# PROBIC/mSWEEP

Hardware: AMD Instinct MI355X
Metric: EM iters/sec + reads×groups cells/sec, 10M reads × 5k groups (higher is better)
Workload: dtype f64

## Files before the change

### msweep_amd/csrc/common.hpp

```cpp
#pragma once
#include <hip/hip_runtime.h>

#include <cstdint>
#include <cstdio>
#include <stdexcept>
#include <string>
#include <vector>

namespace msw {

constexpr int kWave = 64;
#ifndef MSW_PASS_THREADS_A
#define MSW_PASS_THREADS_A 1024
#endif
#ifndef MSW_PASS_THREADS_B
#define MSW_PASS_THREADS_B 768
#endif
#ifndef MSW_PASS_THREADS_B8
#define MSW_PASS_THREADS_B8 1024
#endif
constexpr int kPassThreads = MSW_PASS_THREADS_A;
constexpr int kPassThreadsB = MSW_PASS_THREADS_B;
constexpr int kPassThreadsB8 = MSW_PASS_THREADS_B8;
constexpr int kMaxTrace = 4096;
constexpr int kRedfinParts = 5;
constexpr int kRedfinGroups = 16;
#ifndef MSW_REDFIN_THREADS
#define MSW_REDFIN_THREADS 512
#endif
constexpr int kRedfinThreads = MSW_REDFIN_THREADS;
constexpr int kRedfinSlots = kRedfinThreads / kRedfinGroups;
#ifndef MSW_FX
#define MSW_FX 1
#endif
constexpr bool kFx = MSW_FX != 0;

struct HipError : std::runtime_error {
  using std::runtime_error::runtime_error;
};

#define MSW_HIP(expr)                                                                      \
  do {                                                                                     \
    hipError_t _e = (expr);                                                                \
    if (_e != hipSuccess) {                                                                \
      char _b[512];                                                                        \
      snprintf(_b, sizeof _b, "%s failed: %s (%s:%d)", #expr, hipGetErrorString(_e),       \
               __FILE__, __LINE__);                                                        \
      throw ::msw::HipError(_b);                                                           \
    }                                                                                      \
  } while (0)

template <class T>
struct DevBuf {
  T *p = nullptr;
  size_t n = 0;
  DevBuf() = default;
  DevBuf(const DevBuf &) = delete;
  DevBuf &operator=(const DevBuf &) = delete;
  ~DevBuf() { release(); }
  void release() {
    if (p) (void)hipFree(p);
    p = nullptr;
    n = 0;
  }
  void alloc(size_t count) {
    if (count <= n && p) return;
    release();
    if (count == 0) count = 1;
    MSW_HIP(hipMalloc((void **)&p, count * sizeof(T)));
    n = count;
  }
  void upload(const T *src, size_t count, hipStream_t s) {
    alloc(count);
    if (count) MSW_HIP(hipMemcpyAsync(p, src, count * sizeof(T), hipMemcpyHostToDevice, s));
  }
  void zero(hipStream_t s) {
    if (p) MSW_HIP(hipMemsetAsync(p, 0, n * sizeof(T), s));
  }
};

struct SolveOpts {
  int32_t check_every = 1;
  double init_bound = -100000.0;
  int32_t em_prior = 0;
  int32_t em_stop = 0;
};

#ifdef MSW_STAMPS
__device__ unsigned long long g_stamps[64 * 40];
#define MSW_STAMP(it, K, p) (g_stamps[((it) & 63) * 40 + (K) * 8 + (p)] = __builtin_amdgcn_s_memrealtime())
#define MSW_STAMP_MAX(it, K, p) atomicMax(&g_stamps[((it) & 63) * 40 + (K) * 8 + (p)], (unsigned long long)__builtin_amdgcn_s_memrealtime())
#else
#define MSW_STAMP(it, K, p) ((void)0)
#define MSW_STAMP_MAX(it, K, p) ((void)0)
#endif

struct TabDev {
  double2 *A, *B;
};

struct Scalars {
  double a, os_a, step_a;
  double oldnorm, newnorm, beta;
  double bound, oldbound, bound_const;
  double tol, csum;
  double M, U, p0, kappa;
  double logzi;
  double fx_scale, fx_inv, fx_tscale, fx_tinv, xb, tmax, tmin;
  double tref;
  int32_t didreset, reset_pending, done, iter;
  int32_t have_eval, eval_pad;
  int32_t max_iters, fixed_iters, trace_theta, flavor;
  int32_t check_every, em_prior, em_stop, opt_pad;
  int32_t tab_ver, fx_shift;
};

}
```

### msweep_amd/csrc/msweep_core.hip

```cpp
#include "../../include/msweep_core.h"

#include <algorithm>
#include <array>
#include <cmath>
#include <chrono>
#include <cstring>
#include <limits>
#include <memory>
#include <string>
#include <thread>
#include <unordered_map>
#include <vector>

#include <rocprim/device/device_radix_sort.hpp>
#include <rocprim/device/device_scan.hpp>
#include <rocprim/iterator/counting_iterator.hpp>
#include <rocprim/iterator/transform_iterator.hpp>

#include "kernels.hpp"
#include "pack_kernels.hpp"
#include "compress_kernels.hpp"
#include "comm.hpp"
#include "shm_comm.hpp"
#include "peer_comm.hpp"
#include "likelihood_kernels.hpp"
#include "bootstrap_kernels.hpp"
#include "em_kernels.hpp"
#include "em_f32_kernels.hpp"
#include "stream_kernels.hpp"
#include "reader_kernels.hpp"
#include "bin_kernels.hpp"

using namespace msw;

namespace {
thread_local std::string g_create_error;
constexpr size_t kLdsMax = 160 * 1024;
constexpr int kIterBatch = 16;
}


struct LikShape {
  int flavor = -1;
  uint32_t G = 0, E = 0, n_lut = 0, nslices = 0, n_long = 0;
  uint64_t nnz = 0, nslots = 0;
  int enc = kEncNarrow;
  bool glds = true, tlds = true;
  int gmodeB = 1;
  RecDec dec = {};
  uint32_t n_area = 0;
  uint32_t n_tab_lds = 0;
  SliceClasses cls = {};
  bool packed_scheduled = false;
  uint32_t long_row = kLongRow;
  uint64_t rows_over8 = 0;
  bool passB_rc8 = false;
  double logzi = 0.0;
  int nblk = 0;
  int nblk_dense = 0;
  int nreg = 0;
  bool have_logc_res = false;
};

struct Resident : LikShape {
  DevBuf<uint32_t> rec, slice_off, long_ptr, rec_long, perm;
  DevBuf<uint8_t> slice_hot;
  DevBuf<uint32_t> area_slot;
  DevBuf<double> lut_area;
  DevBuf<double> lut, Lt;
  DevBuf<double> trange;
  DevBuf<double> logc_res;
  bool wide() const { return enc == kEncWide; }
  bool hybrid() const { return enc == kEncIndex; }
  int n_tab_inline() const { return flavor == 0 && n_area <= (uint32_t)kTabInline ? (int)n_area : 0; }
  int npart_rows() const { return flavor == 0 ? nblk : (nreg >= 32 ? 4 * nblk_dense : nblk_dense); }
  uint32_t guard_cap() const {
    static_assert(kPassThreads / 64 <= 16 && kPassThreadsB / 64 <= 16, "guard_cap / guard_bits assume <= 16 wavefronts per workgroup");
    const uint32_t nb0 = (uint32_t)std::max(nblk, 1);
    return 64u * ((nslices + nb0 - 1) / nb0 + 16u) + (n_long + nb0 - 1) / nb0 + 16u;
  }
  uint32_t guard_words() const { return (G + 31u) / 32u; }
};

struct Solver {
  hipStream_t stream = nullptr;
  int n_cu = 256;
  msw_comm *const *commp;
  bool *collective;
  explicit Solver(msw_comm *const *c = nullptr, bool *coll = nullptr) : commp(c), collective(coll) {}
  msw_comm *comm() const { return commp ? *commp : nullptr; }
  SolveOpts opts;
  bool profiling = false, fixed_iters = false;
  size_t trace_theta = 0;

  DevBuf<double> cvec, logc_d, alpha0, u, os_u, step_u, w, e, N, Nc, Acc;
  DevBuf<uint8_t> c8, c8s;
  DevBuf<double2> ew, tabA, tabB;
  TabDev tabs() const { return TabDev{tabA.p, tabB.p}; }
  DevBuf<int> tab_built;
  DevBuf<double> partA, partS, partAcc, partC, partR, totS;
  size_t lds_attr[3][80] = {};
  DevBuf<double> commA, commB;
  DevBuf<uint32_t> guard_list, guard_bits;
  DevBuf<unsigned long long> guard_tail;
  DevBuf<int> guard_err;
  DevBuf<unsigned long long> guard_visits;
  DevBuf<Scalars> sc;
  Scalars *sc_host = nullptr;
  DevBuf<double> tr_bound, tr_newnorm, tr_beta, tr_theta;
  DevBuf<int32_t> tr_reset;
  bool have_solution = false;
  bool prepared = false;
  int last_algo = MSW_ALGO_RCG;
  DevBuf<double> logth;
  DevBuf<float> e32, tab32;
  bool em_f32 = false;

  msw_timing timing = {};
  hipEvent_t ev0 = nullptr, ev1 = nullptr;
  std::vector<std::pair<hipEvent_t, hipEvent_t>> evA, evB, evC;
  size_t evA_used = 0, evB_used = 0, evC_used = 0;

  ~Solver() {
    if (sc_host) (void)hipHostFree(sc_host);
    if (ev0) (void)hipEventDestroy(ev0);
    if (ev1) (void)hipEventDestroy(ev1);
    for (auto &p : evA) { (void)hipEventDestroy(p.first); (void)hipEventDestroy(p.second); }
    for (auto &p : evB) { (void)hipEventDestroy(p.first); (void)hipEventDestroy(p.second); }
    for (auto &p : evC) { (void)hipEventDestroy(p.first); (void)hipEventDestroy(p.second); }
  }
};

struct Resampler {
  DevBuf<uint64_t> mtwords;
  DevBuf<uint32_t> bcounts, bcounts2;
  DevBuf<MtState> mt;
  hipStream_t stream2 = nullptr;
  hipEvent_t ev_counts[2] = {nullptr, nullptr};
  uint32_t one_count = 0;
  bool mt_valid = false;
  int32_t mt_seed = 0;
  uint64_t mt_pos = 0;
  ~Resampler() {
    for (auto &e : ev_counts)
      if (e) (void)hipEventDestroy(e);
    if (stream2) (void)hipStreamDestroy(stream2);
  }
};

struct Worker {
  Solver s;
  Resampler r;
  explicit Worker(int n_cu) { MSW_HIP(hipStreamCreateWithFlags(&s.stream, hipStreamNonBlocking)); s.n_cu = n_cu; }
  ~Worker() { (void)hipStreamDestroy(s.stream); }
};

struct msw_core {
  int device = 0;
  int n_cu = 256;
  hipStream_t stream = nullptr;
  std::string err;
  TextStager text_stage;
  ReaderPool reader_pool;
  msw_comm *comm = nullptr;
  bool in_collective = false;
  bool pack_schedule = true;
  bool no_hybrid = false;

  Resident lik;
  DevBuf<uint32_t> iperm;
  Solver solver{&comm, &in_collective};

  DevBuf<double> cp;
  std::vector<uint32_t> cp_counts;
  bool cp_hit = false;
  Resampler resampler;
  std::vector<std::unique_ptr<Worker>> workers;
  msw_bootstrap_timing btiming = {};

  ~msw_core() { if (stream) (void)hipStreamDestroy(stream); }
};

namespace {

struct Fail : std::runtime_error {
  using std::runtime_error::runtime_error;
};
struct NumericFail : Fail {
  using Fail::Fail;
};

struct CollectiveScope {
  bool *flag;
  explicit CollectiveScope(bool *f) : flag(f) { if (flag) *flag = true; }
  void leave() { if (flag) *flag = false; }
};

template <class F>
int guarded(msw_handle h, F &&f) {
  if (!h) return 1;
  try {
    MSW_HIP(hipSetDevice(h->device));
    f();
    return 0;
  } catch (const std::exception &ex) {
    h->err = ex.what();
    (void)hipGetLastError();
    if (h->comm && h->in_collective) h->comm->abort();
    h->in_collective = false;
    return 1;
  }
}

std::pair<hipEvent_t, hipEvent_t> &next_pair(std::vector<std::pair<hipEvent_t, hipEvent_t>> &v,
                                             size_t &used) {
  if (used == v.size()) {
    hipEvent_t a, b;
    MSW_HIP(hipEventCreate(&a));
    MSW_HIP(hipEventCreate(&b));
    v.emplace_back(a, b);
  }
  return v[used++];
}

SellDev sell_view(const Resident &L, const Solver &s) {
  SellDev S;
  S.rec = L.rec.p;
  S.slice_off = L.slice_off.p;
  S.long_ptr = L.long_ptr.p;
  S.rec_long = L.rec_long.p;
  S.perm = L.perm.p;
  S.cvec = s.cvec.p;
  S.c8 = s.c8.p;
  S.c8s = s.c8s.p;
  S.nslices = L.nslices;
  S.n_long = L.n_long;
  S.n_ecs = L.E;
  S.n_groups = L.G;
  S.n_lut = L.n_lut;
  S.n_area = L.n_area;
  S.area_slot = L.area_slot.p;
  S.shift = L.dec.shift;
  S.mask = L.dec.mask;
  S.bhi = L.dec.bhi;
  S.bhiA = L.dec.bhiA;
  S.shiftH = L.dec.shiftH;
  S.maskH = L.dec.maskH;
  S.n_tab_lds = L.n_tab_lds;
  S.slice_hot = L.slice_hot.p;
  S.lut_area = L.lut_area.p;
  S.cls = L.cls;
  return S;
}
GuardDev guard_view(const Resident &L, const Solver &s) {
  return GuardDev{s.guard_list.p, s.guard_bits.p, s.guard_tail.p, L.lut_area.p, s.guard_err.p, s.guard_visits.p, L.guard_cap(),
                  L.guard_words()};
}

int passB_mode(const Resident &L, bool glds, uint32_t n_tab, bool index) {
  const uint32_t G = L.G;
  if (glds) {
    if (pass_lds_bytes(1, n_tab, G, false, index) > kLdsMax) return -1;
    if (8ull * (G + kSentinels) <= kAccFixed && pass_lds_bytes(2, n_tab, G, false, index) <= kLdsMax) return 2;
    return 1;
  }
  if (pass_lds_bytes(0, n_tab, G, false, index) > kLdsMax) return -1;
  if (getenv("MSWEEP_GLOBAL_ATOMICS")) return 0;
  if (pass_lds_bytes(3, n_tab, G, false, index) <= kLdsMax) return 3;
  if (pass_lds_bytes(4, n_tab, G, false, index) <= kLdsMax) return 4;
  return 0;
}

bool multilane() {
  const char *e = getenv("MSWEEP_MULTILANE");
  return !(e && atoi(e) == 0);
}
SliceClasses make_slice_classes(const uint32_t *n) {
  SliceClasses C = {};
  for (int c = 0; c < kSliceClasses; ++c) {
    const uint32_t per = 64u >> (kMaxLgm - c);
    C.p0[c + 1] = C.p0[c] + n[c];
    C.s0[c + 1] = C.s0[c] + (n[c] + per - 1) / per;
  }
  return C;
}

void choose_lds_mode(Resident &L) {
  const bool opts[4][2] = {{true, true}, {true, false}, {false, true}, {false, false}};
  const char *force = getenv("MSWEEP_FORCE_LDS");
  for (auto &o : opts) {
    if (force && strlen(force) == 2 && (o[0] != (force[0] == '1') || o[1] != (force[1] == '1'))) continue;
    const uint32_t n_tab = o[1] ? L.n_area : 0u;
    const int gmB = passB_mode(L, o[0], n_tab, false);
    if (!force && !o[0] && o[1] && gmB == 0 && !getenv("MSWEEP_GLOBAL_ATOMICS")) continue;
    if (gmB >= 0 && pass_lds_bytes(o[0] ? 1 : 0, n_tab, L.G, true, false) <= kLdsMax) {
      L.glds = o[0];
      L.tlds = o[1];
      L.gmodeB = gmB;
      L.n_tab_lds = n_tab;
      return;
    }
  }
  throw Fail("internal: no LDS configuration fits");
}

void choose_layout(Resident &L) {
  choose_lds_mode(L);
  L.dec.bhi = sell_bhi(L.n_tab_lds);
  L.dec.bhiA = 2 * L.dec.bhi;
  const uint64_t lo_end = 16ull * std::max<uint32_t>(L.n_area, 1);
  const uint64_t hi_end = (uint64_t)L.dec.bhi + 8ull * ((uint64_t)L.G + kSentinels);
  L.enc = kEncWide;
  L.dec.shift = 0;
  L.dec.mask = 0xffffffffu;
  const char *force = getenv("MSWEEP_RECORD_BYTES");
  for (uint32_t s = 5; s <= 31 && !(force && atoi(force) == 8); ++s) {
    if (lo_end <= (1ull << (s - 1)) && hi_end <= (1ull << (32 - s))) {
      L.enc = kEncNarrow;
      L.dec.shift = s;
      L.dec.mask = (1u << (s - 1)) - 1u;
      break;
    }
  }
  if (L.wide() && (hi_end > (1ull << 31) || lo_end > (1ull << 32)))
    throw Fail("likelihood too large: group / lookup-table offsets exceed the 8-byte record fields");
}

bool choose_hybrid_layout(Resident &L, bool no_hybrid) {
  if (L.tlds || no_hybrid) return false;
  if (const char *e = getenv("MSWEEP_HYBRID"))
    if (atoi(e) == 0) return false;
  const char *force = getenv("MSWEEP_RECORD_BYTES");
  if (force && atoi(force) == 8) return false;
  uint32_t eb = 1, gb = 1;
  while ((1ull << eb) < std::max<uint32_t>(L.n_area, 2)) ++eb;
  while ((1ull << gb) < (uint64_t)L.G + kSentinels) ++gb;
  if (eb + gb > 32) return false;
  uint32_t n_hot = 0;
  {
    const int gmA = L.glds ? 1 : 0;
    uint32_t lo = 0, hi = std::min<uint32_t>(L.n_area, (uint32_t)(kLdsMax / 16)) / 16;
    while (lo < hi) {
      const uint32_t mid = (lo + hi + 1) / 2, n = mid * 16;
      const bool ok = pass_lds_bytes(gmA, n, L.G, true, true) <= kLdsMax && passB_mode(L, L.glds, n, true) >= 0 &&
                      (L.glds || passB_mode(L, false, n, true) == passB_mode(L, false, 0, true));
      if (ok) lo = mid;
      else hi = mid - 1;
    }
    n_hot = lo * 16;
  }
  if (const char *e = getenv("MSWEEP_HYBRID_HOT")) n_hot = std::min<uint32_t>(n_hot, (uint32_t)atoi(e) & ~15u);
  L.enc = kEncIndex;
  L.dec.shift = eb;
  L.dec.mask = (1u << eb) - 1u;
  L.n_tab_lds = std::min(n_hot, L.n_area);
  uint32_t hb = 4;
  while ((1ull << hb) < 16ull * std::max<uint32_t>(L.n_tab_lds, 1)) ++hb;
  if (hb + gb > 32) return false;
  L.dec.shiftH = hb;
  L.dec.maskH = (1u << hb) - 1u;
  L.dec.bhi = L.dec.bhiA = sell_bhi(L.n_tab_lds);
  L.gmodeB = passB_mode(L, L.glds, L.n_tab_lds, true);
  return true;
}

void alloc_solve_state(const Resident &L, Solver &s) {
  const uint32_t G = L.G, E = L.E;
  for (DevBuf<double> *b : {&s.alpha0, &s.u, &s.os_u, &s.step_u, &s.w, &s.e, &s.N, &s.Nc,
                            &s.Acc, &s.logth})
    b->alloc((size_t)G + kSentinels);
  s.ew.alloc((size_t)G + kSentinels);
  s.e.zero(s.stream);
  s.ew.zero(s.stream);
  s.cvec.alloc(E);
  s.c8.alloc((size_t)E + 64);
  s.c8s.alloc((size_t)L.nslices * 64 + 64);
  s.c8s.zero(s.stream);
  s.logc_d.alloc(E);
  s.tabA.alloc((size_t)std::max<uint32_t>(L.n_area, 1));
  s.tabB.alloc((size_t)std::max<uint32_t>(L.n_area, 1));
  s.tab_built.alloc(2);
  const int nb = std::max(L.nblk, std::max(L.nblk_dense, L.npart_rows()));
  s.partA.alloc(std::max(nb, 1024));
  s.partS.alloc(4 * (size_t)std::max(nb, 1024));
  s.partR.alloc(kRedfinParts * ((size_t)G / kRedfinGroups + 2));
  s.totS.alloc(4);
  s.commA.alloc(1);
  s.commB.alloc(3 * (size_t)G + 4);
  s.partAcc.alloc((size_t)std::max(nb, 1) * G);
  s.partC.alloc(1024);
  if (L.flavor == 0) {
    const uint32_t nb0 = (uint32_t)std::max(L.nblk, 1);
    s.guard_list.alloc((size_t)nb0 * L.guard_cap());
    s.guard_bits.alloc((size_t)nb0 * 16 * L.guard_words());
    s.guard_bits.zero(s.stream);
    s.guard_tail.alloc(2 * (size_t)G);
    s.guard_tail.zero(s.stream);
  }
  s.guard_err.alloc(1);
  s.guard_err.zero(s.stream);
  s.guard_visits.alloc(1);
  s.guard_visits.zero(s.stream);
  s.sc.alloc(1);
  s.tr_bound.alloc(kMaxTrace);
  s.tr_newnorm.alloc(kMaxTrace);
  s.tr_beta.alloc(kMaxTrace);
  s.tr_reset.alloc(kMaxTrace);
  if (!s.sc_host) MSW_HIP(hipHostMalloc((void **)&s.sc_host, sizeof(Scalars)));
  if (!s.ev0) {
    MSW_HIP(hipEventCreate(&s.ev0));
    MSW_HIP(hipEventCreate(&s.ev1));
  }
}

template <class K>
void prepare_sweep(K k, size_t lds, size_t &lds_set) {
  if (lds > lds_set) {
    hipFuncAttributes fa;
    MSW_HIP(hipFuncGetAttributes(&fa, (const void *)k));
    if (fa.sharedSizeBytes != 0) throw Fail("internal: sweep kernel owns static LDS");
    MSW_HIP(hipFuncSetAttribute((const void *)k, hipFuncAttributeMaxDynamicSharedMemorySize, (int)lds));
    lds_set = lds;
  }
}
template <int ENC, bool GL, bool TL>
void launch_passA_t(const Resident &L, Solver &s) {
  const size_t lds = pass_lds_bytes(GL ? 1 : 0, L.n_tab_lds, L.G, true, ENC == kEncIndex);
  const bool ml = L.cls.s0[kSliceClasses - 1] > 0;
  auto k = ml ? k_passA<ENC, GL, TL, true> : k_passA<ENC, GL, TL, false>;
  prepare_sweep(k, lds, s.lds_attr[0][(ml ? 40 : 0) + ENC * 4 + (GL ? 2 : 0) + (TL ? 1 : 0)]);
  hipLaunchKernelGGL(k, dim3(L.nblk), dim3(pass_threads_A<ENC>()), lds, s.stream, s.sc.p, sell_view(L, s),
                     s.ew.p, s.tabA.p, s.partA.p, s.partR.p, (int)((L.G + kRedfinGroups - 1) / kRedfinGroups),
                     guard_view(L, s));
}
template <int ENC, int GM, bool TL>
void launch_passB_t(const Resident &L, Solver &s) {
  const size_t lds = pass_lds_bytes(GM, L.n_tab_lds, L.G, false, ENC == kEncIndex);
  const bool ml = L.cls.s0[kSliceClasses - 1] > 0;
  if constexpr (ENC == kEncNarrow) {
    if (L.passB_rc8 && !ml) {
      auto k8 = k_passB<ENC, GM, TL, false, 8>;
      prepare_sweep(k8, lds, s.lds_attr[2][2 * GM + (TL ? 1 : 0)]);
      const auto rg_of = [&](uint32_t g0) {
        return GM == 4 ? RangeB{g0, std::min<uint32_t>(kRangeGroups, L.G - g0), g0 == 0 ? 1 : 0} : RangeB{0, 0, 1};
      };
      for (uint32_t g0 = 0; g0 < (GM == 4 ? L.G : 1u); g0 += kRangeGroups)
        hipLaunchKernelGGL(k8, dim3(L.nblk), dim3(pass_threads_B<ENC, 8>()), lds, s.stream, s.sc.p, sell_view(L, s), s.e.p,
                           s.tabB.p, s.partAcc.p, s.partS.p, s.Acc.p, rg_of(g0), guard_view(L, s));
      return;
    }
  }
  auto k = ml ? k_passB<ENC, GM, TL, true> : k_passB<ENC, GM, TL, false>;
  prepare_sweep(k, lds, s.lds_attr[1][(ml ? 40 : 0) + ENC * 10 + 2 * GM + (TL ? 1 : 0)]);
  if (GM == 4) {
    for (uint32_t g0 = 0; g0 < L.G; g0 += kRangeGroups)
      hipLaunchKernelGGL(k, dim3(L.nblk), dim3(pass_threads_B<ENC>()), lds, s.stream, s.sc.p, sell_view(L, s), s.e.p,
                         s.tabB.p, s.partAcc.p, s.partS.p, s.Acc.p,
                         RangeB{g0, std::min<uint32_t>(kRangeGroups, L.G - g0), g0 == 0 ? 1 : 0}, guard_view(L, s));
    return;
  }
  hipLaunchKernelGGL(k, dim3(L.nblk), dim3(pass_threads_B<ENC>()), lds, s.stream, s.sc.p, sell_view(L, s), s.e.p,
                     s.tabB.p, s.partAcc.p, s.partS.p, s.Acc.p, RangeB{0, 0, 1}, guard_view(L, s));
}

#define MSW_DISPATCH3(fn, ...)                                                       \
  do {                                                                               \
    const int key = L.enc * 4 + (L.glds ? 2 : 0) + (L.tlds ? 1 : 0);              \
    switch (key) {                                                                   \
      case 0: fn<kEncNarrow, false, false>(__VA_ARGS__); break;                      \
      case 1: fn<kEncNarrow, false, true>(__VA_ARGS__); break;                       \
      case 2: fn<kEncNarrow, true, false>(__VA_ARGS__); break;                       \
      case 3: fn<kEncNarrow, true, true>(__VA_ARGS__); break;                        \
      case 4: fn<kEncWide, false, false>(__VA_ARGS__); break;                        \
      case 5: fn<kEncWide, false, true>(__VA_ARGS__); break;                         \
      case 6: fn<kEncWide, true, false>(__VA_ARGS__); break;                         \
      case 7: fn<kEncWide, true, true>(__VA_ARGS__); break;                          \
      case 8: fn<kEncIndex, false, false>(__VA_ARGS__); break;                       \
      case 10: fn<kEncIndex, true, false>(__VA_ARGS__); break;                       \
      case 12: fn<kEncValue, false, false>(__VA_ARGS__); break;                      \
      case 14: fn<kEncValue, true, false>(__VA_ARGS__); break;                       \
      default: throw Fail("internal: no sweep for this layout");                     \
    }                                                                                \
  } while (0)
#define MSW_DISPATCH_B(fn, ...)                                                      \
  do {                                                                               \
    const int key = L.enc * 10 + 2 * L.gmodeB + (L.tlds ? 1 : 0);                 \
    switch (key) {                                                                   \
      case 0: fn<kEncNarrow, 0, false>(__VA_ARGS__); break;                          \
      case 1: fn<kEncNarrow, 0, true>(__VA_ARGS__); break;                           \
      case 2: fn<kEncNarrow, 1, false>(__VA_ARGS__); break;                          \
      case 3: fn<kEncNarrow, 1, true>(__VA_ARGS__); break;                           \
      case 4: fn<kEncNarrow, 2, false>(__VA_ARGS__); break;                          \
      case 5: fn<kEncNarrow, 2, true>(__VA_ARGS__); break;                           \
      case 6: fn<kEncNarrow, 3, false>(__VA_ARGS__); break;                          \
      case 7: fn<kEncNarrow, 3, true>(__VA_ARGS__); break;                           \
      case 8: fn<kEncNarrow, 4, false>(__VA_ARGS__); break;                          \
      case 9: fn<kEncNarrow, 4, true>(__VA_ARGS__); break;                           \
      case 10: fn<kEncWide, 0, false>(__VA_ARGS__); break;                           \
      case 11: fn<kEncWide, 0, true>(__VA_ARGS__); break;                            \
      case 12: fn<kEncWide, 1, false>(__VA_ARGS__); break;                           \
      case 13: fn<kEncWide, 1, true>(__VA_ARGS__); break;                            \
      case 14: fn<kEncWide, 2, false>(__VA_ARGS__); break;                           \
      case 15: fn<kEncWide, 2, true>(__VA_ARGS__); break;                            \
      case 16: fn<kEncWide, 3, false>(__VA_ARGS__); break;                           \
      case 17: fn<kEncWide, 3, true>(__VA_ARGS__); break;                            \
      case 18: fn<kEncWide, 4, false>(__VA_ARGS__); break;                           \
      case 19: fn<kEncWide, 4, true>(__VA_ARGS__); break;                            \
      case 20: fn<kEncIndex, 0, false>(__VA_ARGS__); break;                          \
      case 22: fn<kEncIndex, 1, false>(__VA_ARGS__); break;                          \
      case 24: fn<kEncIndex, 2, false>(__VA_ARGS__); break;                          \
      case 26: fn<kEncIndex, 3, false>(__VA_ARGS__); break;                          \
      case 28: fn<kEncIndex, 4, false>(__VA_ARGS__); break;                          \
      case 30: fn<kEncValue, 0, false>(__VA_ARGS__); break;                          \
      case 32: fn<kEncValue, 1, false>(__VA_ARGS__); break;                          \
      case 34: fn<kEncValue, 2, false>(__VA_ARGS__); break;                          \
      case 36: fn<kEncValue, 3, false>(__VA_ARGS__); break;                          \
      case 38: fn<kEncValue, 4, false>(__VA_ARGS__); break;                          \
      default: throw Fail("internal: no sweep for this layout");                     \
    }                                                                                \
  } while (0)

template <int NREG>
void launch_dense_A(const Resident &L, Solver &s) {
  hipLaunchKernelGGL(k_dense_passA<NREG>, dim3(L.nblk_dense), dim3(256), 0, s.stream, s.sc.p,
                     L.Lt.p, (int)L.G, L.E, s.u.p, s.w.p, s.partA.p);
}
template <int NREG>
void launch_dense_B(const Resident &L, Solver &s) {
  const size_t lds = (32 + 4 * (size_t)L.G) * sizeof(double);
  hipLaunchKernelGGL(k_dense_passB<NREG>, dim3(L.nblk_dense), dim3(256), lds, s.stream, s.sc.p,
                     L.Lt.p, (int)L.G, L.E, s.cvec.p, s.u.p, s.partAcc.p, s.partS.p);
}
template <int NREG>
void launch_dense_big_A(const Resident &L, Solver &s) {
  hipLaunchKernelGGL(k_dense_big_passA<NREG>, dim3(L.nblk_dense), dim3(256), 0, s.stream, s.sc.p,
                     L.Lt.p, (int)L.G, L.E, s.u.p, s.w.p, s.partA.p);
}
template <int NREG>
void launch_dense_big_B(const Resident &L, Solver &s) {
  hipLaunchKernelGGL(k_dense_big_passB<NREG>, dim3(L.nblk_dense), dim3(256), 0, s.stream, s.sc.p,
                     L.Lt.p, (int)L.G, L.E, s.cvec.p, s.u.p, s.partAcc.p, s.partS.p);
}
#define MSW_DISPATCH_NREG(fn, fnbig, ...)                \
  do {                                                   \
    switch (L.nreg) {                                   \
      case 1: fn<1>(__VA_ARGS__); break;                 \
      case 2: fn<2>(__VA_ARGS__); break;                 \
      case 4: fn<4>(__VA_ARGS__); break;                 \
      case 8: fn<8>(__VA_ARGS__); break;                 \
      case 16: fn<16>(__VA_ARGS__); break;               \
      case 32: fnbig<32>(__VA_ARGS__); break;            \
      case 64: fnbig<64>(__VA_ARGS__); break;            \
      default: fnbig<128>(__VA_ARGS__); break;           \
    }                                                    \
  } while (0)

void launch_passA(const Resident &L, Solver &s) {
  std::pair<hipEvent_t, hipEvent_t> *ev = nullptr;
  if (s.profiling) {
    ev = &next_pair(s.evA, s.evA_used);
    MSW_HIP(hipEventRecord(ev->first, s.stream));
  }
  if (L.flavor == 0) MSW_DISPATCH3(launch_passA_t, L, s);
  else MSW_DISPATCH_NREG(launch_dense_A, launch_dense_big_A, L, s);
  MSW_HIP(hipGetLastError());
  if (ev) MSW_HIP(hipEventRecord(ev->second, s.stream));
  s.timing.passA_launches++;
}

bool em_f32_layout_ok(const Resident &L, const Solver &s) {
  if (!kFx || L.flavor != 0 || !L.glds || s.comm() || L.G > (uint32_t)(kStepRegs * 1024)) return false;
  if (getenv("MSWEEP_EM_FLOAT_AS_DOUBLE")) return false;
  if (L.enc == kEncNarrow)
    return L.tlds && L.n_tab_lds == L.n_area && em_f32_lds_bytes(L.n_tab_lds, L.G) <= kLdsMax;
  if (L.hybrid()) return L.dec.shift <= 30 && em_f32_idx_lds_bytes(L.n_area, L.G) <= kLdsMax;
  return false;
}
void launch_em_passB_f32(const Resident &L, Solver &s) {
  const bool idx = L.hybrid();
  const size_t lds = idx ? em_f32_idx_lds_bytes(L.n_area, L.G) : em_f32_lds_bytes(L.n_tab_lds, L.G);
  const bool ml = L.cls.s0[kSliceClasses - 1] > 0;
  auto k = idx ? (ml ? k_em_passB_f32_idx<true> : k_em_passB_f32_idx<false>)
               : (ml ? k_em_passB_f32<true> : k_em_passB_f32<false>);
  prepare_sweep(k, lds, s.lds_attr[2][30 + (idx ? 2 : 0) + (ml ? 1 : 0)]);
  hipLaunchKernelGGL(k, dim3(L.nblk), dim3(1024), lds, s.stream, s.sc.p, sell_view(L, s), s.e.p, s.e32.p, s.tab32.p,
                     s.partAcc.p, s.partS.p, guard_view(L, s));
}

void launch_passB(const Resident &L, Solver &s) {
  std::pair<hipEvent_t, hipEvent_t> *ev = nullptr;
  if (s.profiling) {
    ev = &next_pair(s.evB, s.evB_used);
    MSW_HIP(hipEventRecord(ev->first, s.stream));
  }
  if (L.flavor == 0 && s.em_f32) {
    launch_em_passB_f32(L, s);
  } else if (L.flavor == 0) {
    if (L.gmodeB == 0) MSW_HIP(hipMemsetAsync(s.Acc.p, 0, ((size_t)L.G + kSentinels) * sizeof(double), s.stream));
    MSW_DISPATCH_B(launch_passB_t, L, s);
  } else {
    MSW_DISPATCH_NREG(launch_dense_B, launch_dense_big_B, L, s);
  }
  MSW_HIP(hipGetLastError());
  if (ev) MSW_HIP(hipEventRecord(ev->second, s.stream));
  s.timing.passB_launches++;
  const bool partials = (L.flavor == 1) || L.gmodeB > 0 || s.em_f32;
  const int nb = L.npart_rows();
  const int fxrows = L.flavor == 0 ? (s.em_f32 ? 2 : 1) : 0;
  if (s.comm()) {
    const size_t G3 = 3 * (size_t)L.G;
    std::pair<hipEvent_t, hipEvent_t> *evc = nullptr;
    if (s.profiling) {
      evc = &next_pair(s.evC, s.evC_used);
      MSW_HIP(hipEventRecord(evc->first, s.stream));
    }
    hipLaunchKernelGGL(k_colsum, dim3((L.G + 63) / 64), dim3(1024), 0, s.stream, s.sc.p, (int)L.G,
                       partials ? nb : 0, fxrows, nb, s.partAcc.p, s.Acc.p, s.partS.p,
                       fxrows ? s.guard_tail.p : nullptr, s.commB.p);
    if (kFx && fxrows) {
      s.comm()->allreduce_mixed(reinterpret_cast<uint64_t *>(s.commB.p), G3, s.commB.p + G3, 4, s.stream);
    } else {
      s.comm()->allreduce(s.commB.p, (size_t)L.G, s.stream);
      s.comm()->allreduce_mixed(reinterpret_cast<uint64_t *>(s.commB.p) + L.G, 2 * (size_t)L.G, s.commB.p + G3, 4,
                               s.stream);
    }
    if (evc) MSW_HIP(hipEventRecord(evc->second, s.stream));
    hipLaunchKernelGGL(k_redfin, dim3((L.G + kRedfinGroups - 1) / kRedfinGroups), dim3(kRedfinThreads), 0, s.stream,
                       s.sc.p, (int)L.G, 0, fxrows, reinterpret_cast<unsigned long long *>(s.commB.p) + L.G, 0, 1,
                       s.partAcc.p, s.commB.p, s.commB.p + G3, s.e.p, s.u.p,
                       s.alpha0.p, s.Nc.p, s.N.p, s.w.p, s.ew.p, s.partR.p, s.totS.p);
    return;
  }
  hipLaunchKernelGGL(k_redfin, dim3((L.G + kRedfinGroups - 1) / kRedfinGroups), dim3(kRedfinThreads), 0, s.stream,
                     s.sc.p, (int)L.G, partials ? nb : 0, fxrows, fxrows ? s.guard_tail.p : nullptr, 1, nb,
                     s.partAcc.p, s.Acc.p, s.partS.p, s.e.p,
                     s.u.p, s.alpha0.p, s.Nc.p, s.N.p, s.w.p, s.ew.p, s.partR.p, s.totS.p);
}

const double *fin_partS(const Resident &L, Solver &s) { return s.comm() ? s.commB.p + 3 * (size_t)L.G : s.partS.p; }
int fin_npartS(const Resident &L, Solver &s) { return s.comm() ? 1 : L.npart_rows(); }

void launch_tables(const Resident &L, Solver &s) {
  if (L.flavor != 0 || L.n_area <= (uint32_t)kTabInline) return;
  const unsigned nb = std::min<unsigned>((L.n_area + 255) / 256, (unsigned)s.n_cu * 8);
  hipLaunchKernelGGL(k_tables, dim3(nb), dim3(256), 0, s.stream, s.sc.p, (int)L.n_area, L.lut_area.p, s.tabs(),
                     s.tab_built.p);
}

void launch_finstep(const Resident &L, Solver &s, int mode) {
  TraceDev tr{s.tr_bound.p, s.tr_newnorm.p, s.tr_beta.p, s.tr_theta.p, s.tr_reset.p};
  const double *pA = s.partA.p;
  int npA = L.flavor == 0 ? L.nblk : L.nblk_dense;
  if (s.comm()) {
    pA = s.commA.p;
    npA = 1;
  }
  hipLaunchKernelGGL(k_finstep, dim3(1), dim3(1024), 0, s.stream, s.sc.p, mode, (int)L.G, L.n_tab_inline(), npA, pA,
                     (int)((L.G + kRedfinGroups - 1) / kRedfinGroups), s.totS.p, s.partR.p, s.Nc.p, s.w.p, s.u.p,
                     s.os_u.p, s.step_u.p, L.lut_area.p, s.e.p, s.tabs(), tr);
  launch_tables(L, s);
}

void poll(Solver &s) {
  MSW_HIP(hipMemcpyAsync(s.sc_host, s.sc.p, sizeof(Scalars), hipMemcpyDeviceToHost, s.stream));
  MSW_HIP(hipStreamSynchronize(s.stream));
  if (s.comm()) s.comm()->check();
}

constexpr int kCvecBlocks = 512;
void prepare_inputs(const Resident &L, Solver &s, const double *logc_host, const uint32_t *counts_dev,
                    const double *alpha0_host) {
  if (L.flavor < 0) throw Fail("no likelihood resident: call msw_core_set_csr / set_dense_logl first");
  const uint32_t E = L.E, G = L.G;
  if (counts_dev) {
    hipLaunchKernelGGL(k_cvec_from_counts, dim3(kCvecBlocks), dim3(256), 0, s.stream, counts_dev,
                       L.flavor == 0 ? L.perm.p : nullptr, E, s.cvec.p, s.c8.p, s.partC.p, L.cls, L.n_long,
                       L.flavor == 0 ? s.c8s.p : nullptr);
  } else {
    const double *src = s.logc_d.p;
    if (logc_host) {
      MSW_HIP(hipMemcpyAsync(s.logc_d.p, logc_host, E * sizeof(double), hipMemcpyHostToDevice, s.stream));
    } else {
      if (!L.have_logc_res) throw Fail("null logc: only a likelihood built by msw_core_build_likelihood keeps its log counts");
      src = L.logc_res.p;
    }
    hipLaunchKernelGGL(k_cvec_from_logc, dim3(kCvecBlocks), dim3(256), 0, s.stream, src,
                       L.flavor == 0 ? L.perm.p : nullptr, E, s.cvec.p, s.c8.p, s.partC.p, L.cls, L.n_long,
                       L.flavor == 0 ? s.c8s.p : nullptr);
  }
  if (alpha0_host)
    MSW_HIP(hipMemcpyAsync(s.alpha0.p, alpha0_host, G * sizeof(double), hipMemcpyHostToDevice, s.stream));
  MSW_HIP(hipGetLastError());
  MSW_HIP(hipStreamSynchronize(s.stream));
  s.prepared = true;
}

void validate_solve(size_t max_iters, int algo, int prec) {
  if (algo != MSW_ALGO_RCG && algo != MSW_ALGO_EM) throw Fail("unknown algorithm id");
  if (prec != MSW_PREC_DOUBLE && prec != MSW_PREC_FLOAT) throw Fail("unknown precision id");
  if (max_iters == 0 || max_iters > (size_t)std::numeric_limits<int32_t>::max())
    throw Fail("max_iters out of range");
}

void begin_solve(const Resident &L, Solver &s, double tol, size_t max_iters) {
  const uint32_t G = L.G;
  if (s.trace_theta) s.tr_theta.alloc(s.trace_theta * G);
  const double *cpart = s.partC.p;
  int ncpart = kCvecBlocks;
  if (s.comm()) {
    s.comm()->rendezvous();
    hipLaunchKernelGGL(k_sum_scalar, dim3(1), dim3(1024), 0, s.stream, s.sc.p, 0, kCvecBlocks, s.partC.p,
                       s.commA.p);
    s.comm()->allreduce(s.commA.p, 1, s.stream);
    cpart = s.commA.p;
    ncpart = 1;
  }
  hipLaunchKernelGGL(k_init_state, dim3(1), dim3(1024), 0, s.stream, s.sc.p, (int)G, ncpart,
                     cpart, s.alpha0.p, s.u.p, s.os_u.p, s.step_u.p, tol, (int)max_iters,
                     s.fixed_iters ? 1 : 0, (int)s.trace_theta, L.flavor, L.logzi, s.opts, s.tab_built.p,
                     L.trange.p);
  MSW_HIP(hipGetLastError());
}

void run_rcg(const Resident &L, Solver &s, size_t max_iters, size_t iters_start = 0) {
  const int G = (int)L.G, n_lut = L.n_tab_inline();
  if (iters_start > 0 && s.comm()) s.comm()->rendezvous();
  if (iters_start == 0) {
    hipLaunchKernelGGL(k_prepB, dim3(1), dim3(1024), 0, s.stream, s.sc.p, G, n_lut, s.u.p, L.lut_area.p,
                       s.e.p, s.tabs());
    launch_tables(L, s);
    launch_passB(L, s);
    s.timing.passB_launches--;
    if (s.profiling && s.evB_used) s.evB_used--;
  }
  const int nbA = L.flavor == 0 ? L.nblk : L.nblk_dense;
  size_t iters_done = iters_start;
  for (;;) {
    const size_t missing = std::max<size_t>(1, max_iters - std::min(max_iters, iters_done));
    const size_t batch = s.fixed_iters ? std::min<size_t>(256, missing) : std::min<size_t>(kIterBatch, missing);
    for (size_t b = 0; b < batch; ++b) {
      launch_passA(L, s);
      if (s.comm()) {
        std::pair<hipEvent_t, hipEvent_t> *evc = nullptr;
        if (s.profiling) {
          evc = &next_pair(s.evC, s.evC_used);
          MSW_HIP(hipEventRecord(evc->first, s.stream));
        }
        hipLaunchKernelGGL(k_sum_scalar, dim3(1), dim3(1024), 0, s.stream, s.sc.p, 1, nbA, s.partA.p,
                           s.commA.p);
        s.comm()->allreduce(s.commA.p, 1, s.stream);
        if (evc) MSW_HIP(hipEventRecord(evc->second, s.stream));
      }
      launch_finstep(L, s, 0);
      launch_passB(L, s);
    }
    MSW_HIP(hipGetLastError());
    poll(s);
    if (s.sc_host->done) break;
    if (s.sc_host->have_eval && (size_t)s.sc_host->iter + 1 >= max_iters) {
      launch_finstep(L, s, 1);
      MSW_HIP(hipGetLastError());
      poll(s);
      if (s.sc_host->done) break;
    }
    iters_done = (size_t)s.sc_host->iter;
  }
}

void finish_solve(const Resident &L, Solver &s, double *theta_out, size_t *iters_out, double *bound_out) {
  poll(s);
  const uint32_t G = L.G;
  int gerr = 0;
  MSW_HIP(hipMemcpy(&gerr, s.guard_err.p, sizeof gerr, hipMemcpyDeviceToHost));
  if (gerr) {
    MSW_HIP(hipMemset(s.guard_err.p, 0, sizeof gerr));
    if (gerr == 2) throw Fail("internal: a workgroup's list of guarded equivalence classes overflowed");
    throw NumericFail("likelihood underflow: an equivalence class has zero probability under every group "
                      "(exp(a * log-likelihood) and the group weights underflow fp64 together)");
  }
  if (s.sc_host->iter > 0 && !std::isfinite(s.sc_host->bound))
    throw NumericFail("the evidence lower bound is not finite: the likelihood or the prior counts are out of range");
  if (theta_out) {
    if (s.last_algo == MSW_ALGO_EM) {
      MSW_HIP(hipMemcpy(theta_out, s.logth.p, G * sizeof(double), hipMemcpyDeviceToHost));
    } else {
      std::vector<double> nc(G);
      MSW_HIP(hipMemcpy(nc.data(), s.Nc.p, G * sizeof(double), hipMemcpyDeviceToHost));
      const double csum = s.sc_host->csum;
      for (uint32_t g = 0; g < G; ++g) theta_out[g] = nc[g] / csum;
    }
  }
  if (iters_out) *iters_out = (size_t)s.sc_host->iter;
  if (bound_out) *bound_out = s.sc_host->bound;
  s.have_solution = true;
}

void collect_timing(const Resident &L, Solver &s) {
  float ms = 0.f;
  MSW_HIP(hipEventElapsedTime(&ms, s.ev0, s.ev1));
  s.timing.solve_ms = ms;
  s.timing.passA_ms = s.timing.passB_ms = 0.0;
  if (s.profiling) {
    for (size_t i = 0; i < s.evA_used; ++i) {
      MSW_HIP(hipEventElapsedTime(&ms, s.evA[i].first, s.evA[i].second));
      s.timing.passA_ms += ms;
    }
    for (size_t i = 0; i < s.evB_used; ++i) {
      MSW_HIP(hipEventElapsedTime(&ms, s.evB[i].first, s.evB[i].second));
      s.timing.passB_ms += ms;
    }
    s.timing.collective_ms = 0.0;
    for (size_t i = 0; i < s.evC_used; ++i) {
      MSW_HIP(hipEventElapsedTime(&ms, s.evC[i].first, s.evC[i].second));
      s.timing.collective_ms += ms;
    }
    s.timing.collectives = s.evC_used;
  }
  s.timing.iters = (uint64_t)s.sc_host->iter;
  const uint64_t recsz = L.enc == kEncValue ? 12 : (L.wide() ? 8 : 4);
  if (L.flavor == 0) {
    const uint64_t tab = L.tlds ? 0ull : 16ull * (L.n_area - L.n_tab_lds);
    s.timing.bytes_passA = L.nnz * recsz + tab;
    s.timing.bytes_passB = L.nnz * recsz + 1ull * L.E + tab;
  } else {
    s.timing.bytes_passA = 8ull * L.E * L.G;
    s.timing.bytes_passB = 8ull * L.E * L.G + 8ull * L.E;
  }
}

void run_em(const Resident &L, Solver &s, size_t max_iters, int prec);

void continue_impl(const Resident &L, Solver &s, size_t n_iters, double *theta_out, size_t *iters_out, double *bound_out) {
  if (!s.have_solution || !s.fixed_iters || s.last_algo != MSW_ALGO_RCG)
    throw Fail("msw_core_continue: needs a fixed-iteration RCG solve on the handle (msw_core_set_fixed_iters, msw_core_run)");
  const size_t start = (size_t)s.sc_host->iter;
  if (n_iters == 0 || start + n_iters > (size_t)std::numeric_limits<int32_t>::max()) throw Fail("msw_core_continue: iteration count out of range");
  s.timing = {};
  s.evA_used = s.evB_used = s.evC_used = 0;
  CollectiveScope cs(s.collective);
  hipLaunchKernelGGL(k_extend, dim3(1), dim3(1), 0, s.stream, s.sc.p, (int)n_iters);
  MSW_HIP(hipEventRecord(s.ev0, s.stream));
  run_rcg(L, s, start + n_iters, start);
  MSW_HIP(hipEventRecord(s.ev1, s.stream));
  finish_solve(L, s, theta_out, iters_out, bound_out);
  collect_timing(L, s);
  s.timing.iters = (uint64_t)s.sc_host->iter - start;
  cs.leave();
}

void run_impl(const Resident &L, Solver &s, double tol, size_t max_iters, int algo, int prec, double *theta_out,
              size_t *iters_out, double *bound_out) {
  validate_solve(max_iters, algo, prec);
  if (!s.prepared) throw Fail("msw_core_run: inputs not prepared (call msw_core_prepare)");
  s.timing = {};
  s.evA_used = s.evB_used = s.evC_used = 0;
  CollectiveScope cs(s.collective);
  begin_solve(L, s, tol, max_iters);
  MSW_HIP(hipEventRecord(s.ev0, s.stream));
  if (algo == MSW_ALGO_RCG) run_rcg(L, s, max_iters);
  else run_em(L, s, max_iters, prec);
  MSW_HIP(hipEventRecord(s.ev1, s.stream));
  s.last_algo = algo;
  finish_solve(L, s, theta_out, iters_out, bound_out);
  collect_timing(L, s);
  cs.leave();
}

}

namespace {
struct StageTimer {
  hipStream_t st;
  bool on;
  std::chrono::steady_clock::time_point t0;
  explicit StageTimer(hipStream_t s) : st(s), on(getenv("MSWEEP_BUILD_TIMING") != nullptr), t0(std::chrono::steady_clock::now()) {}
  void mark(const char *what) {
    if (!on) return;
    (void)hipStreamSynchronize(st);
    const auto t1 = std::chrono::steady_clock::now();
    fprintf(stderr, "[msweep build] %-28s %8.2f ms\n", what, std::chrono::duration<double, std::milli>(t1 - t0).count());
    t0 = t1;
  }
};
}

#include "host_likelihood.inc"
#include "host_pack.inc"
#include "host_em.inc"
#include "host_mtjump.inc"
#include "host_bootstrap.inc"
#include "host_build.inc"
#include "host_compress.inc"
#include "host_alignment.inc"
#include "host_reader.inc"
#include "host_bin.inc"

extern "C" {

#ifndef MSW_SRC_HASH
#define MSW_SRC_HASH "unhashed"
#endif
const char *msw_core_version(void) { return "msweep_core 0.2 gfx950 (HIP, wave64) src " MSW_SRC_HASH; }

const char *msw_last_error(msw_handle h) { return h ? h->err.c_str() : g_create_error.c_str(); }

int msw_core_create(int device, msw_handle *out) {
  if (!out) return 1;
  *out = nullptr;
  try {
    int n = 0;
    MSW_HIP(hipGetDeviceCount(&n));
    if (n <= 0) throw Fail("no HIP device visible: libmsweep_core has no CPU fallback");
    if (device < 0 || device >= n) throw Fail("device index out of range");
    MSW_HIP(hipSetDevice(device));
    hipDeviceProp_t prop;
    MSW_HIP(hipGetDeviceProperties(&prop, device));
    std::unique_ptr<msw_core> h(new msw_core);
    h->device = device;
    h->n_cu = prop.multiProcessorCount > 0 ? prop.multiProcessorCount : 256;
    MSW_HIP(hipStreamCreateWithFlags(&h->stream, hipStreamNonBlocking));
    h->solver.stream = h->stream;
    h->solver.n_cu = h->n_cu;
    hipLaunchKernelGGL(k_warm, dim3(1), dim3(1), 0, h->stream, (int *)nullptr);
    MSW_HIP(hipGetLastError());
    MSW_HIP(hipStreamSynchronize(h->stream));
    *out = h.release();
    return 0;
  } catch (const std::exception &ex) {
    g_create_error = ex.what();
    (void)hipGetLastError();
    return 1;
  }
}

void msw_core_destroy(msw_handle h) {
  if (!h) return;
  (void)hipSetDevice(h->device);
  if (h->stream) (void)hipStreamSynchronize(h->stream);
  delete h;
}

int msw_core_shape(msw_handle h, size_t *n_groups, size_t *n_ecs, size_t *nnz) {
  return guarded(h, [&] {
    if (h->lik.flavor < 0) throw Fail("no likelihood resident");
    if (n_groups) *n_groups = h->lik.G;
    if (n_ecs) *n_ecs = h->lik.E;
    if (nnz) *nnz = h->lik.flavor == 0 ? h->lik.nnz : (size_t)h->lik.G * h->lik.E;
  });
}

int msw_core_set_dense_logl(msw_handle h, const double *L, size_t n_groups, size_t n_ecs, size_t ld) {
  return guarded(h, [&] { set_dense_impl(h, L, n_groups, n_ecs, ld); });
}

int msw_core_set_csr(msw_handle h, const uint64_t *rowptr, const uint32_t *grp, const uint32_t *cnt,
                     const double *lut, size_t lut_ld, double logzi, size_t n_groups, size_t n_ecs) {
  return guarded(h, [&] { set_csr_impl(h, rowptr, grp, cnt, lut, lut_ld, logzi, n_groups, n_ecs); });
}

int msw_core_build_likelihood(msw_handle h, const uint64_t *ec_tptr, const uint32_t *ec_targets,
                              size_t n_ecs, const uint32_t *target_group, size_t n_targets,
                              const uint64_t *group_sizes, size_t n_groups, const uint64_t *ec_counts,
                              double q, double e, double zero_inflation, size_t min_hits,
                              size_t *n_groups_out, uint8_t *mask_out, double *logc_out) {
  return guarded(h, [&] {
    build_likelihood_impl(h, ec_tptr, ec_targets, n_ecs, target_group, n_targets, group_sizes,
                          n_groups, ec_counts, q, e, zero_inflation, min_hits, n_groups_out, mask_out,
                          logc_out, false, 0);
  });
}

int msw_core_build_likelihood_aln(msw_handle h, msw_alignment_t a, const uint32_t *target_group, size_t n_targets,
                                  const uint64_t *group_sizes, size_t n_groups, double q, double e,
                                  double zero_inflation, size_t min_hits, size_t *n_groups_out, uint8_t *mask_out,
                                  double *logc_out) {
  return guarded(h, [&] {
    if (!a) throw Fail("msw_core_build_likelihood_aln: null alignment");
    if (a->on_device && a->device == h->device) {
      build_likelihood_impl(h, a->d_tptr.p, a->d_targets.p, a->E, target_group, n_targets, group_sizes, n_groups,
                            a->d_counts.p, q, e, zero_inflation, min_hits, n_groups_out, mask_out, logc_out, true, a->H);
    } else {
      a->to_host(msw_alignment::kAlnTptr | msw_alignment::kAlnTargets | msw_alignment::kAlnCounts);
      build_likelihood_impl(h, a->ec_tptr.data(), a->ec_targets.data(), a->ec_counts.size(), target_group, n_targets,
                            group_sizes, n_groups, a->ec_counts.data(), q, e, zero_inflation, min_hits, n_groups_out,
                            mask_out, logc_out, false, 0);
    }
  });
}

int msw_core_trim(msw_handle h) {
  return guarded(h, [&] {
    MSW_HIP(hipStreamSynchronize(h->stream));
    h->reader_pool.trim();
  });
}

int msw_alignment_read_device(msw_handle h, const char *const *paths, size_t n_paths, size_t n_targets, int merge_mode,
                              msw_alignment_t *out) {
  if (out) *out = nullptr;
  const int rc = guarded(h, [&] {
    check_reader_args(paths, out, n_paths, n_targets, merge_mode);
    std::unique_ptr<msw_alignment> a(new msw_alignment);
    a->device = h->device;
    MSW_HIP(hipStreamSynchronize(h->stream));
    h->reader_pool.recycle();
    ReaderCtx cx(h->stream, h->n_cu, &h->text_stage, &h->reader_pool, h->device);
    bool fits = true;
    {
      uint64_t text = 0;
      for (size_t i = 0; i < n_paths; ++i) {
        struct stat sb;
        if (paths[i] && stat(paths[i], &sb) == 0) text += (uint64_t)sb.st_size * (path_is_gzip(paths[i]) ? 8u : 1u);
      }
      size_t free_b = 0, total_b = 0;
      MSW_HIP(hipMemGetInfo(&free_b, &total_b));
      const uint64_t need = 6 * text + (1ull << 30);
      if (need > (uint64_t)free_b && h->reader_pool.idle_bytes()) {
        h->reader_pool.trim();
        MSW_HIP(hipMemGetInfo(&free_b, &total_b));
      }
      fits = need <= (uint64_t)free_b + h->reader_pool.idle_bytes();
      if (getenv("MSWEEP_READER_FORCE_HOST")) fits = false;
    }
    try {
      if (!fits) throw ReaderFallback{};
      try {
        read_alignment_device(paths, n_paths, n_targets, merge_mode, cx, *a);
      } catch (const HipError &ex) {
        if (!strstr(ex.what(), "out of memory")) throw;
        (void)hipGetLastError();
        throw ReaderFallback{};
      }
    } catch (const ReaderFallback &) {
      msw_alignment_t host = nullptr;
      if (msw_alignment_read(paths, n_paths, n_targets, merge_mode, &host) != 0) throw Fail(msw_alignment_last_error());
      *out = host;
      return;
    }
    *out = a.release();
  });
  if (rc != 0 && h) g_aln_error = msw_last_error(h);
  return rc;
}

int msw_core_layout_info(msw_handle h, msw_layout_info *out) {
  return guarded(h, [&] {
    if (!out) throw Fail("null out");
    const Resident &L = h->lik;
    if (L.flavor != 0) throw Fail("msw_core_layout_info: no CSR-of-ECs likelihood resident");
    msw_layout_info li = {};
    li.record_bytes = L.enc == kEncValue ? 12 : (L.wide() ? 8 : 4);
    li.index_records = L.hybrid() ? 1 : 0;
    li.groups_in_lds = L.glds ? 1 : 0;
    li.table_in_lds = L.tlds ? 1 : 0;
    li.passB_mode = L.gmodeB;
    li.slot_entries = L.n_area;
    li.slot_entries_in_lds = L.n_tab_lds;
    li.n_slices = L.nslices;
    li.n_long_ecs = L.n_long;
    li.bank_scheduled = L.packed_scheduled ? 1 : 0;
    li.passB_reg_cells = L.passB_rc8 ? 8 : kRegCells;
    li.rows_over_8 = L.rows_over8;
    std::vector<uint32_t> off((size_t)L.nslices + 1);
    MSW_HIP(hipMemcpy(off.data(), L.slice_off.p, off.size() * sizeof(uint32_t), hipMemcpyDeviceToHost));
    li.rows = off[L.nslices];
    for (int c = 0; c < kSliceClasses; ++c) li.slices_by_lanes[c] = L.cls.s0[c + 1] - L.cls.s0[c];
    for (uint32_t s2 = 0; s2 < L.nslices; ++s2) li.max_rows = std::max(li.max_rows, off[s2 + 1] - off[s2]);
    if (L.hybrid()) {
      std::vector<uint8_t> hot(std::max<uint32_t>(L.nslices, 1));
      MSW_HIP(hipMemcpy(hot.data(), L.slice_hot.p, hot.size(), hipMemcpyDeviceToHost));
      for (uint32_t s2 = 0; s2 < L.nslices; ++s2) li.rows_from_memory += (off[s2 + 1] - off[s2]) - hot[s2];
    } else if (!L.tlds && L.enc != kEncValue) {
      li.rows_from_memory = li.rows;
    }
    *out = li;
  });
}

int msw_core_layout_hash(msw_handle h, uint64_t *hash_out) {
  return guarded(h, [&] {
    if (!hash_out) throw Fail("null out");
    *hash_out = layout_hash(h->lik);
  });
}

int msw_core_get_dense_logl(msw_handle h, double *L_out, size_t ld) {
  return guarded(h, [&] { materialise_impl(h, L_out, ld, false, 0, h->lik.E); });
}

int msw_core_gamma(msw_handle h, double *gamma_out, size_t ld) {
  return guarded(h, [&] {
    if (!h->solver.have_solution) throw Fail("msw_core_gamma: no solve has run on this handle");
    materialise_impl(h, gamma_out, ld, true, 0, h->lik.E);
  });
}

int msw_core_gamma_block(msw_handle h, size_t ec_begin, size_t ec_end, double *gamma_out, size_t ld) {
  return guarded(h, [&] {
    if (!h->solver.have_solution) throw Fail("msw_core_gamma_block: no solve has run on this handle");
    materialise_impl(h, gamma_out, ld, true, ec_begin, ec_end);
  });
}

int msw_core_bin_reads(msw_handle h, const uint64_t *ec_rptr, const uint32_t *ec_reads, size_t n_ecs,
                       const uint32_t *targets, const double *thresholds, size_t n_targets, uint64_t *bin_ptr,
                       uint32_t *reads_out, double *log_thr_out) {
  return guarded(h, [&] {
    bin_reads_impl(h, ec_rptr, ec_reads, n_ecs, false, targets, thresholds, n_targets, bin_ptr, reads_out, log_thr_out);
  });
}

int msw_core_bin_reads_aln(msw_handle h, msw_alignment_t a, const uint32_t *targets, const double *thresholds,
                           size_t n_targets, uint64_t *bin_ptr, uint32_t *reads_out, double *log_thr_out) {
  return guarded(h, [&] {
    if (!a) throw Fail("msw_core_bin_reads_aln: null alignment");
    if (a->on_device && a->device == h->device) {
      bin_reads_impl(h, a->d_rptr.p, a->d_reads.p, a->E, true, targets, thresholds, n_targets, bin_ptr, reads_out,
                     log_thr_out);
    } else {
      a->to_host(msw_alignment::kAlnRptr | msw_alignment::kAlnReads);
      bin_reads_impl(h, a->ec_rptr.data(), a->ec_reads.data(), a->ec_rptr.empty() ? 0 : a->ec_rptr.size() - 1, false,
                     targets, thresholds, n_targets, bin_ptr, reads_out, log_thr_out);
    }
  });
}

int msw_core_solve(msw_handle h, const double *logc, const double *alpha0, double tol, size_t max_iters,
                   int algo, int prec, double *theta_out, size_t *iters_out, double *bound_out) {
  return guarded(h, [&] {
    if (!alpha0) throw Fail("msw_core_solve: null alpha0");
    prepare_inputs(h->lik, h->solver, logc, nullptr, alpha0);
    run_impl(h->lik, h->solver, tol, max_iters, algo, prec, theta_out, iters_out, bound_out);
  });
}

int msw_core_prepare(msw_handle h, const double *logc, const double *alpha0) {
  return guarded(h, [&] {
    if (!alpha0) throw Fail("msw_core_prepare: null alpha0");
    prepare_inputs(h->lik, h->solver, logc, nullptr, alpha0);
  });
}

int msw_core_run(msw_handle h, double tol, size_t max_iters, int algo, int prec, double *theta_out,
                 size_t *iters_out, double *bound_out) {
  return guarded(h, [&] { run_impl(h->lik, h->solver, tol, max_iters, algo, prec, theta_out, iters_out, bound_out); });
}

int msw_core_continue(msw_handle h, size_t n_iters, double *theta_out, size_t *iters_out, double *bound_out) {
  return guarded(h, [&] { continue_impl(h->lik, h->solver, n_iters, theta_out, iters_out, bound_out); });
}

int msw_core_set_trace_theta(msw_handle h, size_t n_iters) {
  return guarded(h, [&] {
    if (n_iters > (size_t)kMaxTrace) throw Fail("trace_theta: at most 4096 iterations");
    h->solver.trace_theta = n_iters;
  });
}

int msw_core_trace(msw_handle h, size_t n, double *bound, double *newnorm, double *beta,
                   int32_t *didreset, double *theta_trace, size_t *n_out) {
  return guarded(h, [&] {
    if (!h->solver.have_solution) throw Fail("msw_core_trace: no solve has run on this handle");
    size_t have = std::min<size_t>((size_t)h->solver.sc_host->iter, kMaxTrace);
    n = std::min(n, have);
    if (bound) MSW_HIP(hipMemcpy(bound, h->solver.tr_bound.p, n * sizeof(double), hipMemcpyDeviceToHost));
    if (newnorm) MSW_HIP(hipMemcpy(newnorm, h->solver.tr_newnorm.p, n * sizeof(double), hipMemcpyDeviceToHost));
    if (beta) MSW_HIP(hipMemcpy(beta, h->solver.tr_beta.p, n * sizeof(double), hipMemcpyDeviceToHost));
    if (didreset) MSW_HIP(hipMemcpy(didreset, h->solver.tr_reset.p, n * sizeof(int32_t), hipMemcpyDeviceToHost));
    if (theta_trace) {
      const size_t nt = std::min(n, h->solver.trace_theta);
      if (nt) MSW_HIP(hipMemcpy(theta_trace, h->solver.tr_theta.p, nt * h->lik.G * sizeof(double), hipMemcpyDeviceToHost));
    }
    if (n_out) *n_out = n;
  });
}

int msw_core_bootstrap(msw_handle h, const uint32_t *ec_counts, int32_t seed, size_t bootstrap_count,
                       size_t rep_begin, size_t rep_end, const double *alpha0, double tol,
                       size_t max_iters, int algo, int prec, double *theta_out, size_t *iters_out) {
  return guarded(h, [&] {
    bootstrap_impl(h, ec_counts, seed, bootstrap_count, rep_begin, rep_end, alpha0, tol, max_iters,
                   algo, prec, theta_out, iters_out);
  });
}

int msw_core_resample_counts(msw_handle h, const uint32_t *ec_counts, size_t n_ecs, int32_t seed,
                             size_t bootstrap_count, size_t rep_begin, size_t rep_end,
                             uint32_t *counts_out) {
  return guarded(h, [&] {
    resample_impl(h, ec_counts, n_ecs, seed, bootstrap_count, rep_begin, rep_end, counts_out);
  });
}

int msw_core_bootstrap_dist(msw_handle h, msw_comm_t comm, const uint32_t *ec_counts, int32_t seed,
                            size_t bootstrap_count, size_t n_replicates, const double *alpha0, double tol,
                            size_t max_iters, int algo, int prec, double *theta_out, size_t *iters_out) {
  return guarded(h, [&] {
    bootstrap_dist_impl(h, comm, ec_counts, seed, bootstrap_count, n_replicates, alpha0, tol, max_iters, algo,
                        prec, theta_out, iters_out);
  });
}

const char *msw_comm_last_error(void) { return g_create_error.c_str(); }

int msw_comm_size(msw_comm_t c, int *nranks, int *rank) {
  if (!c) {
    g_create_error = "msw_comm_size: null communicator";
    return 1;
  }
  if (nranks) *nranks = c->size();
  if (rank) *rank = c->rank();
  return 0;
}

int msw_comm_rccl_count(msw_comm_t c, int *count) {
  if (!c || !count) {
    g_create_error = "msw_comm_rccl_count: null argument";
    return 1;
  }
  if (const PeerComm *pc = dynamic_cast<const PeerComm *>(c)) c = pc->base.get();
  const RcclComm *rc = dynamic_cast<const RcclComm *>(c);
  *count = rc ? rc->count() : 0;
  return 0;
}

int msw_comm_allgather(msw_comm_t c, const double *send, size_t n, double *recv) {
  if (!c || (n && (!send || !recv))) {
    g_create_error = "msw_comm_allgather: null argument";
    return 1;
  }
  try {
    c->allgather_host(send, n, recv);
    return 0;
  } catch (const std::exception &ex) {
    g_create_error = ex.what();
    (void)hipGetLastError();
    c->abort();
    return 1;
  }
}

int msw_comm_allreduce(msw_comm_t c, uint64_t *ints, size_t ni, double *reals, size_t nr, int repeats, double *ms_per_call) {
  if (!c || (ni && !ints) || (nr && !reals) || repeats < 1) {
    g_create_error = "msw_comm_allreduce: bad arguments";
    return 1;
  }
  hipStream_t st = nullptr;
  try {
    MSW_HIP(hipStreamCreateWithFlags(&st, hipStreamNonBlocking));
    DevBuf<double> buf, work;
    buf.alloc(ni + nr + 1);
    work.alloc(ni + nr + 1);
    if (ni) MSW_HIP(hipMemcpyAsync(buf.p, ints, ni * 8, hipMemcpyHostToDevice, st));
    if (nr) MSW_HIP(hipMemcpyAsync(buf.p + ni, reals, nr * 8, hipMemcpyHostToDevice, st));
    const auto t0 = std::chrono::steady_clock::now();
    for (int k = 0; k < repeats; ++k) {
      MSW_HIP(hipMemcpyAsync(work.p, buf.p, (ni + nr) * 8, hipMemcpyDeviceToDevice, st));
      c->allreduce_mixed(reinterpret_cast<uint64_t *>(work.p), ni, work.p + ni, nr, st);
    }
    MSW_HIP(hipStreamSynchronize(st));
    c->check();
    if (ms_per_call)
      *ms_per_call = std::chrono::duration<double, std::milli>(std::chrono::steady_clock::now() - t0).count() / repeats;
    if (ni) MSW_HIP(hipMemcpyAsync(ints, work.p, ni * 8, hipMemcpyDeviceToHost, st));
    if (nr) MSW_HIP(hipMemcpyAsync(reals, work.p + ni, nr * 8, hipMemcpyDeviceToHost, st));
    MSW_HIP(hipStreamSynchronize(st));
    (void)hipStreamDestroy(st);
    return 0;
  } catch (const std::exception &ex) {
    g_create_error = ex.what();
    (void)hipGetLastError();
    if (st) (void)hipStreamDestroy(st);
    c->abort();
    return 1;
  }
}

int msw_comm_unique_id(unsigned char id_out[128]) {
  static_assert(sizeof(ncclUniqueId) == 128, "ncclUniqueId is 128 bytes");
  ncclUniqueId id;
  const ncclResult_t rc = ncclGetUniqueId(&id);
  if (rc != ncclSuccess) {
    g_create_error = std::string("ncclGetUniqueId: ") + ncclGetErrorString(rc);
    return 1;
  }
  std::memcpy(id_out, &id, 128);
  return 0;
}

int msw_comm_create_rccl(const unsigned char id[128], int rank, int nranks, int device, msw_comm_t *out) {
  if (!out || !id || nranks < 1 || rank < 0 || rank >= nranks) {
    g_create_error = "msw_comm_create_rccl: bad arguments";
    return 1;
  }
  try {
    MSW_HIP(hipSetDevice(device));
    ncclUniqueId uid;
    std::memcpy(&uid, id, 128);
    std::unique_ptr<msw_comm> c(new RcclComm(uid, rank, nranks));
    if (peer_allreduce_requested() && nranks > 1) c.reset(new PeerComm(std::move(c), true));
    *out = c.release();
    return 0;
  } catch (const std::exception &ex) {
    g_create_error = ex.what();
    return 1;
  }
}

int msw_comm_create_local(int nranks, msw_comm_t *out) {
  if (!out || nranks < 1) {
    g_create_error = "msw_comm_create_local: bad arguments";
    return 1;
  }
  try {
    const bool peer = peer_allreduce_requested() && nranks > 1;
    auto grp = std::make_shared<LocalGroup>(nranks);
    for (int r = 0; r < nranks; ++r) out[r] = nullptr;
    for (int r = 0; r < nranks; ++r) {
      std::unique_ptr<msw_comm> c(new LocalComm(grp, r));
      if (peer) c.reset(new PeerComm(std::move(c), false));
      out[r] = c.release();
    }
    return 0;
  } catch (const std::exception &ex) {
    for (int r = 0; r < nranks; ++r) delete out[r];
    g_create_error = ex.what();
    return 1;
  }
}

int msw_comm_create_shm(const char *name, int rank, int nranks, int device, msw_comm_t *out) {
  if (!out || !name || nranks < 1 || rank < 0 || rank >= nranks) {
    g_create_error = "msw_comm_create_shm: bad arguments";
    return 1;
  }
  try {
    MSW_HIP(hipSetDevice(device));
    std::unique_ptr<msw_comm> c(new ShmComm(name, rank, nranks));
    if (peer_allreduce_requested() && nranks > 1) c.reset(new PeerComm(std::move(c), true));
    *out = c.release();
    return 0;
  } catch (const std::exception &ex) {
    g_create_error = ex.what();
    return 1;
  }
}

void msw_comm_destroy(msw_comm_t c) { delete c; }

int msw_core_set_comm(msw_handle h, msw_comm_t comm) {
  return guarded(h, [&] { h->comm = comm; });
}

int msw_core_set_profiling(msw_handle h, int enabled) {
  return guarded(h, [&] { h->solver.profiling = enabled != 0; });
}
int msw_core_set_fixed_iters(msw_handle h, int enabled) {
  return guarded(h, [&] { h->solver.fixed_iters = enabled != 0; });
}
int msw_core_set_pack_schedule(msw_handle h, int enabled) {
  return guarded(h, [&] { h->pack_schedule = enabled != 0; });
}
int msw_core_set_option(msw_handle h, int option, double value) {
  return guarded(h, [&] {
    switch (option) {
      case MSW_OPT_CHECK_EVERY:
        if (!(value >= 1.0 && value <= 65536.0) || value != std::floor(value)) throw Fail("MSW_OPT_CHECK_EVERY: an integer in [1, 65536]");
        h->solver.opts.check_every = (int32_t)value;
        break;
      case MSW_OPT_INIT_BOUND:
        if (std::isnan(value) || value == INFINITY) throw Fail("MSW_OPT_INIT_BOUND: a number below +inf");
        h->solver.opts.init_bound = value;
        break;
      case MSW_OPT_EM_PRIOR:
        if (value != 0.0 && value != 1.0) throw Fail("MSW_OPT_EM_PRIOR: 0 (MAP) or 1 (ML)");
        h->solver.opts.em_prior = (int32_t)value;
        break;
      case MSW_OPT_EM_STOP:
        if (value != 0.0 && value != 1.0) throw Fail("MSW_OPT_EM_STOP: 0 (log-likelihood gain) or 1 (largest move of a weight)");
        h->solver.opts.em_stop = (int32_t)value;
        break;
      default: throw Fail("msw_core_set_option: unknown option id");
    }
  });
}
int msw_core_get_option(msw_handle h, int option, double *value) {
  return guarded(h, [&] {
    if (!value) throw Fail("null out");
    switch (option) {
      case MSW_OPT_CHECK_EVERY: *value = h->solver.opts.check_every; break;
      case MSW_OPT_INIT_BOUND: *value = h->solver.opts.init_bound; break;
      case MSW_OPT_EM_PRIOR: *value = h->solver.opts.em_prior; break;
      case MSW_OPT_EM_STOP: *value = h->solver.opts.em_stop; break;
      default: throw Fail("msw_core_get_option: unknown option id");
    }
  });
}
int msw_core_last_timing(msw_handle h, msw_timing *out) {
  return guarded(h, [&] {
    if (!out) throw Fail("null out");
    *out = h->solver.timing;
  });
}

#ifdef MSW_STAMPS
int msw_debug_stamps(msw_handle h, uint64_t *out, int clear) {
  return guarded(h, [&] {
    MSW_HIP(hipStreamSynchronize(h->stream));
    if (out) MSW_HIP(hipMemcpyFromSymbol(out, HIP_SYMBOL(g_stamps), sizeof(unsigned long long) * 64 * 40));
    if (clear) {
      std::vector<unsigned long long> z(64 * 40, 0);
      MSW_HIP(hipMemcpyToSymbol(HIP_SYMBOL(g_stamps), z.data(), z.size() * sizeof(unsigned long long)));
    }
  });
}
#endif

int msw_core_guarded_visits(msw_handle h, uint64_t *out) {
  return guarded(h, [&] {
    if (!out) throw Fail("null out");
    if (h->lik.flavor != 0) throw Fail("msw_core_guarded_visits: no CSR-of-ECs likelihood resident");
    unsigned long long v = 0;
    MSW_HIP(hipStreamSynchronize(h->stream));
    MSW_HIP(hipMemcpy(&v, h->solver.guard_visits.p, sizeof v, hipMemcpyDeviceToHost));
    *out = v;
  });
}

int msw_core_last_bootstrap_timing(msw_handle h, msw_bootstrap_timing *out) {
  return guarded(h, [&] {
    if (!out) throw Fail("null out");
    *out = h->btiming;
  });
}

int msw_core_hbm_stream_rates(msw_handle h, size_t n_bytes, int reps, double *read_gbs, double *triad_gbs) {
  return guarded(h, [&] {
    if (!read_gbs || !triad_gbs) throw Fail("null out");
    if (n_bytes < (1u << 20) || reps < 1) throw Fail("msw_core_hbm_stream_rates: at least 1 MiB and one repetition");
    const size_t n = n_bytes / sizeof(double2);
    DevBuf<double2> a, b, c;
    DevBuf<double> sink;
    a.alloc(n);
    b.alloc(n);
    c.alloc(n);
    sink.alloc(1);
    MSW_HIP(hipMemsetAsync(a.p, 0, n * sizeof(double2), h->stream));
    MSW_HIP(hipMemsetAsync(b.p, 0, n * sizeof(double2), h->stream));
    MSW_HIP(hipMemsetAsync(c.p, 0, n * sizeof(double2), h->stream));
    hipEvent_t e0, e1;
    MSW_HIP(hipEventCreate(&e0));
    MSW_HIP(hipEventCreate(&e1));
    const int shapes[7][2] = {{256, 512}, {256, 1024}, {512, 256}, {512, 1024}, {1024, 512}, {2048, 1024}, {8192, 1024}};
    double best_r = 0.0, best_t = 0.0;
    for (int r = 0; r < reps + 2; ++r) {
      for (const auto &sh : shapes) {
        float ms = 0.f;
        MSW_HIP(hipEventRecord(e0, h->stream));
        k_stream_read<<<sh[0], sh[1], 0, h->stream>>>(a.p, n, sink.p);
        MSW_HIP(hipEventRecord(e1, h->stream));
        MSW_HIP(hipEventSynchronize(e1));
        MSW_HIP(hipEventElapsedTime(&ms, e0, e1));
        if (r >= 2) best_r = std::max(best_r, (double)(n * sizeof(double2)) / (ms * 1e-3) / 1e9);
        MSW_HIP(hipEventRecord(e0, h->stream));
        k_stream_triad<<<sh[0], sh[1], 0, h->stream>>>(a.p, b.p, c.p, n);
        MSW_HIP(hipEventRecord(e1, h->stream));
        MSW_HIP(hipEventSynchronize(e1));
        MSW_HIP(hipEventElapsedTime(&ms, e0, e1));
        if (r >= 2) best_t = std::max(best_t, (double)(3 * n * sizeof(double2)) / (ms * 1e-3) / 1e9);
      }
    }
    MSW_HIP(hipGetLastError());
    (void)hipEventDestroy(e0);
    (void)hipEventDestroy(e1);
    *read_gbs = best_r;
    *triad_gbs = best_t;
  });
}

}
```

### msweep_amd/csrc/state_kernels.hpp

```cpp
#pragma once
#include "device_util.hpp"

namespace msw {

struct TraceDev {
  double *bound, *newnorm, *beta, *theta;
  int32_t *didreset;
};

__device__ inline void prepB_block(Scalars *sc, double a, int G, int n_lut, const double *u,
                                   const double *lut, double *e, TabDev X, double *sh) {
  const int tid = threadIdx.x, nt = blockDim.x;
  double m = -INFINITY;
  for (int g = tid; g < G; g += nt) m = fmax(m, u[g]);
  const double M = block_max(m, sh);
  double su = 0.0;
  for (int g = tid; g < G; g += nt) {
    const double eg = flush_denormal(exp(u[g] - M));
    e[g] = eg;
    su += eg;
  }
  const double U = block_sum(su, sh);
  const double logzi = sc->logzi, oma = 1.0 - a;
  const double tref = tref_of(a, sc->tmax, sc->tmin);
  const double p0 = exp(a * (logzi - tref));
  const double xtop = 1.0;
  for (int i = tid; i < n_lut; i += nt) {
    const double T = lut[i], x = exp(a * (T - tref));
    X.A[i] = make_double2(x, oma * (T - logzi));
    X.B[i] = make_double2(x - p0, x * T - p0 * logzi);
  }
  if (tid == 0) {
    sc->M = M;
    sc->U = U;
    sc->p0 = p0;
    sc->tref = tref;
    sc->xb = fmax(xtop, p0);
    sc->fx_shift = fx_shift_of(fmax(xtop, p0), p0);
    sc->tab_ver = sc->tab_ver + 1;
  }
}

constexpr int kTabInline = 16384;
__global__ __launch_bounds__(256) void k_tables(const Scalars *sc, int n_tab, const double *lut, TabDev X,
                                               int *built) {
  const int ver = sc->tab_ver;
  if (built[0] != ver) {
    const double a = sc->a, logzi = sc->logzi, oma = 1.0 - a;
    const double tref = tref_of(a, sc->tmax, sc->tmin);
    const double p0 = exp(a * (logzi - tref));
    for (int i = blockIdx.x * blockDim.x + threadIdx.x; i < n_tab; i += gridDim.x * blockDim.x) {
      const double T = lut[i], x = exp(a * (T - tref));
      X.A[i] = make_double2(x, oma * (T - logzi));
      X.B[i] = make_double2(x - p0, x * T - p0 * logzi);
    }
  }
  __syncthreads();
  if (threadIdx.x == 0 && atomicAdd(&built[1], 1) == (int)gridDim.x - 1) {
    built[1] = 0;
    built[0] = ver;
  }
}

__global__ __launch_bounds__(1024) void k_minmax(const double *v, uint64_t n, int pairs, double *out) {
  __shared__ double sh[32];
  double mx = -INFINITY, mn = INFINITY;
  const uint64_t stride = (uint64_t)gridDim.x * blockDim.x;
  if (pairs) {
    for (uint64_t i = (uint64_t)blockIdx.x * blockDim.x + threadIdx.x; i < n; i += stride) {
      mx = fmax(mx, v[2 * i]);
      mn = fmin(mn, v[2 * i + 1]);
    }
  } else {
    for (uint64_t i = (uint64_t)blockIdx.x * blockDim.x + threadIdx.x; i < n; i += stride) {
      mx = fmax(mx, v[i]);
      mn = fmin(mn, v[i]);
    }
  }
  mx = block_max(mx, sh);
  mn = -block_max(-mn, sh);
  if (threadIdx.x == 0) {
    out[2 * blockIdx.x] = mx;
    out[2 * blockIdx.x + 1] = mn;
  }
}

__global__ __launch_bounds__(1024) void k_prepB(Scalars *sc, int G, int n_lut, const double *u,
                                               const double *lut, double *e, TabDev X) {
  __shared__ double sh[32];
  if (sc->done) return;
  if (sc->flavor != 0) return;
  const double a = sc->a;
  __syncthreads();
  prepB_block(sc, a, G, n_lut, u, lut, e, X, sh);
}

constexpr int kStepRegs = 6;
__global__ __launch_bounds__(1024) void k_finstep(Scalars *sc, int mode, int G, int n_lut, int n_partA,
                                                 const double *partA, int npartR, const double *totS,
                                                 const double *partR, const double *Nc, const double *w, double *u,
                                                 double *os_u, double *step_u, const double *lut, double *e, TabDev X,
                                                 TraceDev tr) {
  __shared__ double sh[16 * (kRedfinParts + 1)];
  const int tid = threadIdx.x, nt = blockDim.x;
  const bool inreg = G <= kStepRegs * nt;
  double q[kRedfinParts + 1] = {0.0, 0.0, 0.0, 0.0, 0.0, 0.0};
  for (int b = tid; b < npartR; b += nt)
    for (int i = 0; i < kRedfinParts; ++i) q[i] += partR[kRedfinParts * b + i];
  for (int i = tid; i < n_partA; i += nt) q[kRedfinParts] += partA[i];
  const double s_clogZ = totS[0], s_rH = totS[1];
  double wv[kStepRegs], sv[kStepRegs], uv[kStepRegs];
  if (inreg) {
#pragma unroll
    for (int k = 0; k < kStepRegs; ++k) {
      const int g = tid + k * nt;
      if (g < G) {
        wv[k] = w[g];
        sv[k] = step_u[g];
        uv[k] = u[g];
      }
    }
  }
  const double lt = tid < n_lut ? lut[tid] : 0.0;
  if (tid == 0) MSW_STAMP(sc->iter, 1, 0);
  const Scalars s0 = *sc;
  if (s0.done) return;
  block_sum_fixed<kRedfinParts + 1, 16>(q, sh);
  if (tid == 0) MSW_STAMP(s0.iter, 1, 2);
  const double lg = q[0], mu = q[1], S0 = q[2], S1 = q[3], pnsum = q[5];
  const int flavor = s0.flavor;
  const double logzi = s0.logzi;
  double a = s0.a, os_a = s0.os_a, kappa = s0.kappa, bound = s0.bound;
  int didreset = s0.didreset, it = s0.iter, done = 0;
  bool old_is_step = false;

  if (s0.have_eval == 2) {
    if (flavor == 0) kappa += S1 / S0;
  } else if (s0.have_eval == 1) {
    const int reeval = s0.reset_pending;
    const double coef = (flavor == 0) ? (1.0 - a) : 1.0;
    const double nb = s0.bound_const + s_clogZ + coef * s_rH + mu + lg + (flavor == 0 ? a * s0.tref * s0.csum : 0.0);
    if (!reeval && nb < s0.oldbound) {
      double a2 = a;
      if (s0.beta > 0) {
        a2 = a - os_a;
        if (inreg) {
#pragma unroll
          for (int k = 0; k < kStepRegs; ++k)
            if (tid + k * nt < G) u[tid + k * nt] = uv[k] - os_u[tid + k * nt];
        } else {
          for (int g = tid; g < G; g += nt) u[g] -= os_u[g];
        }
      }
      __syncthreads();
      if (tid == 0) {
        sc->a = a2;
        sc->didreset = 1;
        sc->reset_pending = 1;
        sc->bound = nb;
        sc->have_eval = mode == 1 ? 0 : 1;
      }
      if (flavor == 0) prepB_block(sc, a2, G, n_lut, u, lut, e, X, sh);
      return;
    }
    if (it < s0.trace_theta && tr.theta)
      for (int g = tid; g < G; g += nt) tr.theta[(size_t)it * G + g] = Nc[g] / s0.csum;
    if (!s0.fixed_iters && (nb - s0.oldbound < s0.tol) && !didreset && (s0.check_every <= 1 || (it + 1) % s0.check_every == 0))
      done = 1;
    if (it + 1 >= s0.max_iters) done = 1;
    if (tid == 0 && it < kMaxTrace) {
      tr.bound[it] = nb;
      tr.newnorm[it] = s0.newnorm;
      tr.beta[it] = s0.beta;
      tr.didreset[it] = didreset;
    }
    old_is_step = !reeval;
    if (old_is_step) os_a = s0.step_a;
    if (flavor == 0) kappa += S1 / S0;
    bound = nb;
    it += 1;
  } else if (s0.reset_pending) {
    if (tid == 0) sc->have_eval = 1;
    return;
  }
  if (done || mode == 1) {
    if (old_is_step) {
      if (inreg) {
#pragma unroll
        for (int k = 0; k < kStepRegs; ++k)
          if (tid + k * nt < G) os_u[tid + k * nt] = sv[k];
      } else {
        for (int g = tid; g < G; g += nt) os_u[g] = step_u[g];
      }
    }
    if (tid == 0) {
      sc->os_a = os_a;
      sc->bound = bound;
      sc->kappa = kappa;
      sc->reset_pending = 0;
      sc->iter = it;
      sc->done = done;
      sc->have_eval = 0;
      MSW_STAMP(it, 4, 7);
    }
    return;
  }

  const double newnorm = G == 1 ? 0.0 : pnsum;
  const double ratio = newnorm / s0.oldnorm;
  const double beta = ratio < INFINITY ? ratio : 0.0;
  double step_a = 1.0 - a;
  if (didreset) {
    os_a *= 0.0;
  } else if (beta > 0) {
    os_a *= beta;
    step_a += os_a;
  }
  const double a_new = a + step_a;
  if (!inreg) {
    const double *osrc = old_is_step ? step_u : os_u;
    for (int g = tid; g < G; g += nt) {
      double osu = osrc[g], su = w[g];
      if (didreset) {
        osu *= 0.0;
      } else if (beta > 0) {
        osu *= beta;
        su += osu;
      }
      os_u[g] = osu;
      step_u[g] = su;
      u[g] += su;
    }
    __syncthreads();
    if (tid == 0) {
      sc->a = a_new;
      sc->os_a = os_a;
      sc->step_a = step_a;
      sc->oldnorm = newnorm;
      sc->newnorm = newnorm;
      sc->beta = beta;
      sc->didreset = 0;
      sc->reset_pending = 0;
      sc->bound = bound;
      sc->oldbound = bound;
      sc->kappa = kappa;
      sc->iter = it;
      sc->have_eval = 1;
    }
    if (flavor == 0) prepB_block(sc, a_new, G, n_lut, u, lut, e, X, sh);
    return;
  }
  double m = -INFINITY;
#pragma unroll
  for (int k = 0; k < kStepRegs; ++k) {
    const int g = tid + k * nt;
    if (g < G) {
      double osu = old_is_step ? sv[k] : os_u[g], su = wv[k];
      if (didreset) {
        osu *= 0.0;
      } else if (beta > 0) {
        osu *= beta;
        su += osu;
      }
      uv[k] += su;
      os_u[g] = osu;
      step_u[g] = su;
      u[g] = uv[k];
      m = fmax(m, uv[k]);
    }
  }
  double p0 = 0.0, tref = 0.0;
  if (flavor == 0) {
    const double oma = 1.0 - a_new;
    tref = tref_of(a_new, s0.tmax, s0.tmin);
    p0 = exp(a_new * (logzi - tref));
    for (int i = tid; i < n_lut; i += nt) {
      const double T = i == tid ? lt : lut[i], x = exp(a_new * (T - tref));
      X.A[i] = make_double2(x, oma * (T - logzi));
      X.B[i] = make_double2(x - p0, x * T - p0 * logzi);
    }
  }
  double M = 0.0, U = 0.0;
  if (flavor == 0) {
    M = block_max_fixed<16>(m, sh);
    double su = 0.0;
#pragma unroll
    for (int k = 0; k < kStepRegs; ++k) {
      const int g = tid + k * nt;
      if (g < G) {
        const double eg = flush_denormal(exp(uv[k] - M));
        e[g] = eg;
        su += eg;
      }
    }
    U = block_sum_fixed1<16>(su, sh);
  }
  if (tid == 0) MSW_STAMP(s0.iter, 1, 6);
  if (tid == 0) {
    sc->a = a_new;
    sc->tab_ver = s0.tab_ver + 1;
    sc->os_a = os_a;
    sc->step_a = step_a;
    sc->oldnorm = newnorm;
    sc->newnorm = newnorm;
    sc->beta = beta;
    sc->didreset = 0;
    sc->reset_pending = 0;
    sc->bound = bound;
    sc->oldbound = bound;
    sc->kappa = kappa;
    sc->iter = it;
    sc->have_eval = 1;
    if (flavor == 0) {
      sc->M = M;
      sc->U = U;
      sc->p0 = p0;
      sc->tref = tref;
      sc->xb = 1.0;
      sc->fx_shift = fx_shift_of(1.0, p0);
    }
  }
}

__global__ __launch_bounds__(kRedfinThreads) void k_redfin(const Scalars *sc, int G, int nblk, int fxrows,
                                                unsigned long long *tail, int zero_tail,
                                                int npartS, const double *partAcc, const double *Acc,
                                                const double *partS, const double *e, const double *u,
                                                const double *alpha0, double *Nc, double *N, double *w,
                                                double2 *ew, double *partR, double *totS) {
  __shared__ double sh[48];
  __shared__ double accs[kRedfinSlots][kRedfinGroups];
  const int tid = threadIdx.x, gl = tid & (kRedfinGroups - 1), rs = tid >> 4;
  const int g = blockIdx.x * kRedfinGroups + gl;
  if (tid == 0 && blockIdx.x == 0) MSW_STAMP(sc->iter, 3, 0);
  const Scalars s0 = *sc;
  const bool fx = kFx && fxrows;
  double s = 0.0;
  long long si = 0;
  if (g < G) {
    if (nblk > 0) {
      if (fx) {
        const long long *pi = reinterpret_cast<const long long *>(partAcc);
        for (int b = rs; b < nblk; b += kRedfinSlots) si += pi[(size_t)b * G + g];
      } else {
        for (int b = rs; b < nblk; b += kRedfinSlots) s += partAcc[(size_t)b * G + g];
      }
    } else if (rs == 0) {
      if (fx) si = reinterpret_cast<const long long *>(Acc)[g];
      else s = Acc[g];
    }
  }
  if (fx) s = __longlong_as_double(si);
  const bool mathlane = (tid & 63) < kRedfinGroups && tid < 128 && g < G;
  const int role = tid >> 6;
  double ug0 = 0.0, eg0 = 0.0, al0 = 0.0;
  long long th = 0, tl = 0;
  if (mathlane) {
    ug0 = u[g];
    eg0 = e[g];
    al0 = alpha0[g];
    if (tail) {
      th = (long long)tail[2 * (size_t)g];
      tl = (long long)tail[2 * (size_t)g + 1];
    }
  }
  double t[3] = {0.0, 0.0, 0.0};
  for (int b = tid; b < npartS; b += kRedfinThreads) {
    t[0] += partS[4 * b];
    t[1] += partS[4 * b + 1];
    t[2] += partS[4 * b + 2];
  }
  if (s0.done) return;
  if (tail && zero_tail && mathlane && role == 0 && (th | tl)) {
    tail[2 * (size_t)g] = 0;
    tail[2 * (size_t)g + 1] = 0;
  }
  accs[rs][gl] = s;
  if (tid == 0 && blockIdx.x == 0) MSW_STAMP(s0.iter, 3, 1);
  block_sum_fixed<3, kRedfinThreads / 64>(t, sh);
  if (tid == 0 && blockIdx.x == 0) MSW_STAMP(s0.iter, 3, 2);
  const double W = t[2];
  if (blockIdx.x == 0 && tid == 0) {
    totS[0] = t[0];
    totS[1] = t[1];
    totS[2] = t[2];
  }
  if (tid >= 128) return;
  double lgv = 0.0, muv = 0.0, s0v = 0.0, s1v = 0.0, s2v = 0.0;
  if (mathlane) {
    double A = 0.0;
    long long ai = 0;
    if (fx) {
#pragma unroll
      for (int i = 0; i < kRedfinSlots; ++i) ai += __double_as_longlong(accs[i][gl]);
    } else {
#pragma unroll
      for (int i = 0; i < kRedfinSlots; ++i) A += accs[i][gl];
    }
    double nc;
    const double ug = ug0;
    const int flavor = s0.flavor;
    if (flavor == 0 && fx) {
      const double fg = fxrows == 2 ? (eg0 > 0.0 ? eg0 : 1.0) : fx_factor(eg0, fx_expbits(s0.fx_shift));
      const double t1 = fg * (s0.p0 * W) * s0.fx_scale;
      const double th1 = floor(t1 * 0x1p-32), tl1 = fma(-th1, 0x1p32, t1);
      const unsigned long long b =
          ((unsigned long long)(uint32_t)__double2loint(th1 + 6755399441055744.0) << 32) + (unsigned long long)__double2ll_rn(tl1);
      const long long tot = (long long)((unsigned long long)ai + b);
      nc = fmax((double)tot * s0.fx_inv * (eg0 / fg), 0.0);
      nc += (double)th * s0.fx_tinv + (double)tl * (s0.fx_tinv * 0x1p-36);
      muv = (s0.M - ug) * nc;
    } else if (flavor == 0) {
      nc = eg0 * (s0.p0 * W + A);
      nc += (double)th * s0.fx_tinv + (double)tl * (s0.fx_tinv * 0x1p-36);
      muv = (s0.M - ug) * nc;
    } else {
      nc = A;
    }
    const double n = al0 + nc;
    if (role == 0) {
      Nc[g] = nc;
      N[g] = n;
      lgv = lgamma(n);
    } else {
      muv = 0.0;
      const double wg = digamma_ref(n) - 1.0 - ug;
      w[g] = wg;
      if (flavor == 0) {
        const double eg = eg0, wc = wg - s0.kappa;
        const double sb = wc;
        ew[g] = make_double2(eg, wc);
        s0v = eg;
        s1v = eg * sb;
        s2v = eg * sb * sb;
      }
    }
  }
  double *o = partR + kRedfinParts * blockIdx.x;
  if (role == 0) {
    lgv = wave_sum(lgv);
    muv = wave_sum(muv);
    if (tid == 0) {
      o[0] = lgv;
      o[1] = muv;
    }
  } else {
    s0v = wave_sum(s0v);
    s1v = wave_sum(s1v);
    s2v = wave_sum(s2v);
    if (tid == 64) {
      MSW_STAMP_MAX(s0.iter, 3, 7);
      o[2] = s0v;
      o[3] = s1v;
      o[4] = s2v;
    }
  }
}

__global__ __launch_bounds__(1024) void k_sum_scalar(const Scalars *sc, int gate, int n, const double *part,
                                                    double *out) {
  __shared__ double sh[32];
  if (gate && sc->done) return;
  double p = 0.0;
  for (int i = threadIdx.x; i < n; i += blockDim.x) p += part[i];
  p = block_sum(p, sh);
  if (threadIdx.x == 0) out[0] = p;
}

__global__ __launch_bounds__(1024) void k_colsum(const Scalars *sc, int G, int nrows, int fxrows, int npartS,
                                                const double *partAcc, const double *Acc,
                                                const double *partS, unsigned long long *tail, double *out) {
  __shared__ double sh[32];
  __shared__ double accs[16][64];
  if (sc->done) return;
  const int tid = threadIdx.x, lane = tid & 63, wv = tid >> 6;
  const int g = blockIdx.x * 64 + lane;
  if (blockIdx.x == 0) {
    double p1 = 0.0, p2 = 0.0, p3 = 0.0;
    for (int b = tid; b < npartS; b += 1024) {
      p1 += partS[4 * b];
      p2 += partS[4 * b + 1];
      p3 += partS[4 * b + 2];
    }
    p1 = block_sum(p1, sh);
    p2 = block_sum(p2, sh);
    p3 = block_sum(p3, sh);
    if (tid == 0) {
      out[3 * (size_t)G] = p1;
      out[3 * (size_t)G + 1] = p2;
      out[3 * (size_t)G + 2] = p3;
      out[3 * (size_t)G + 3] = 0.0;
    }
  }
  if (wv == 1 && g < G) {
    unsigned long long *o = reinterpret_cast<unsigned long long *>(out) + G;
    const unsigned long long a0 = tail ? tail[2 * (size_t)g] : 0ull, a1 = tail ? tail[2 * (size_t)g + 1] : 0ull;
    o[2 * (size_t)g] = a0;
    o[2 * (size_t)g + 1] = a1;
    if (a0 | a1) {
      tail[2 * (size_t)g] = 0;
      tail[2 * (size_t)g + 1] = 0;
    }
  }
  const bool fx = kFx && fxrows;
  double s = 0.0;
  long long si = 0;
  if (g < G) {
    if (nrows > 0) {
      if (fx) {
        const long long *pi = reinterpret_cast<const long long *>(partAcc);
        for (int b = wv; b < nrows; b += 16) si += pi[(size_t)b * G + g];
      } else {
        for (int b = wv; b < nrows; b += 16) s += partAcc[(size_t)b * G + g];
      }
    } else if (wv == 0) {
      if (fx) si = reinterpret_cast<const long long *>(Acc)[g];
      else s = Acc[g];
    }
  }
  accs[wv][lane] = fx ? __longlong_as_double(si) : s;
  __syncthreads();
  if (wv == 0 && g < G) {
    if (fx) {
      long long ai = 0;
#pragma unroll
      for (int i = 0; i < 16; ++i) ai += __double_as_longlong(accs[i][lane]);
      out[g] = __longlong_as_double(ai);
    } else {
      double A = 0.0;
#pragma unroll
      for (int i = 0; i < 16; ++i) A += accs[i][lane];
      out[g] = A;
    }
  }
}

__device__ __forceinline__ uint8_t c8_of(double &c) {
  const double r = rint(c);
  if (r >= 0.0 && r < 255.0 && fabs(c - r) <= 1e-12 * r) {
    c = r;
    return (uint8_t)r;
  }
  return (uint8_t)255;
}

__device__ __forceinline__ void c8_to_lanes(uint8_t *c8s, const SliceClasses &cls, uint32_t n_long, uint32_t j, uint8_t b) {
  if (!c8s || j < n_long) return;
  uint32_t s, lgm, l0;
  slice_of_position(cls, j - n_long, s, lgm, l0);
  for (uint32_t i = 0; i < (1u << lgm); ++i) c8s[(size_t)s * 64 + l0 + i] = b;
}

__global__ __launch_bounds__(256) void k_cvec_from_logc(const double *logc, const uint32_t *perm,
                                                       uint32_t E, double *cvec, uint8_t *c8, double *part,
                                                       SliceClasses cls, uint32_t n_long, uint8_t *c8s) {
  __shared__ double sh[32];
  double s = 0.0;
  for (uint32_t j = blockIdx.x * blockDim.x + threadIdx.x; j < E; j += gridDim.x * blockDim.x) {
    double c = exp(logc[perm ? perm[j] : j]);
    c8[j] = c8_of(c);
    c8_to_lanes(c8s, cls, n_long, j, c8[j]);
    cvec[j] = c;
    s += c;
  }
  s = block_sum(s, sh);
  if (threadIdx.x == 0) part[blockIdx.x] = s;
}

__global__ __launch_bounds__(256) void k_cvec_from_counts(const uint32_t *cnt, const uint32_t *perm,
                                                         uint32_t E, double *cvec, uint8_t *c8, double *part,
                                                         SliceClasses cls, uint32_t n_long, uint8_t *c8s) {
  __shared__ double sh[32];
  double s = 0.0;
  for (uint32_t j = blockIdx.x * blockDim.x + threadIdx.x; j < E; j += gridDim.x * blockDim.x) {
    double c = (double)cnt[perm ? perm[j] : j];
    c8[j] = c8_of(c);
    c8_to_lanes(c8s, cls, n_long, j, c8[j]);
    cvec[j] = c;
    s += c;
  }
  s = block_sum(s, sh);
  if (threadIdx.x == 0) part[blockIdx.x] = s;
}

__global__ void k_extend(Scalars *sc, int n) {
  sc->max_iters += n;
  sc->done = 0;
}

__global__ __launch_bounds__(1024) void k_init_state(Scalars *sc, int G, int npart, const double *part,
                                                    const double *alpha0, double *u, double *os_u,
                                                    double *step_u, double tol, int max_iters,
                                                    int fixed_iters, int trace_theta, int flavor,
                                                    double logzi, SolveOpts so, int *tab_built,
                                                    const double *trange) {
  const double init_bound = so.init_bound;
  __shared__ double sh[32];
  const int tid = threadIdx.x, nt = blockDim.x;
  double s = 0.0;
  for (int i = tid; i < npart; i += nt) s += part[i];
  const double csum = block_sum(s, sh);
  double sa = 0.0, sl = 0.0;
  for (int g = tid; g < G; g += nt) {
    sa += alpha0[g];
    sl += lgamma(alpha0[g]);
    u[g] = 0.0;
    os_u[g] = 0.0;
    step_u[g] = 0.0;
  }
  sa = block_sum(sa, sh);
  sl = block_sum(sl, sh);
  if (tid == 0) {
    Scalars z = {};
    z.a = 0.0;
    z.oldnorm = 1.0;
    z.bound = init_bound;
    z.oldbound = init_bound;
    z.bound_const = lgamma(sa) - lgamma(sa + csum) - sl;
    z.tol = tol;
    z.csum = csum;
    z.logzi = logzi;
    z.max_iters = max_iters;
    z.fixed_iters = fixed_iters;
    z.trace_theta = trace_theta;
    z.flavor = flavor;
    int ex = 0;
    frexp(csum > 1.0 ? csum : 1.0, &ex);
    const int k = 61 - ex < 120 ? 61 - ex : 120;
    const int t = 50 - ex;
    z.fx_scale = ldexp(1.0, k);
    z.fx_inv = ldexp(1.0, -k);
    z.fx_tscale = ldexp(1.0, t);
    z.fx_tinv = ldexp(1.0, -t);
    z.tmax = fmax(trange[0], logzi);
    z.tmin = fmin(trange[1], logzi);
    z.xb = 1.0;
    z.tref = 0.0;
    z.fx_shift = 9;
    z.have_eval = 2;
    z.check_every = so.check_every < 1 ? 1 : so.check_every;
    z.em_prior = so.em_prior;
    z.em_stop = so.em_stop;
    *sc = z;
    tab_built[0] = -1;
    tab_built[1] = 0;
  }
}

}
```

### msweep_amd/csrc/sweep_kernels.hpp

```cpp
#pragma once
#include <type_traits>

#include "device_util.hpp"
#include "sell.hpp"

namespace msw {

constexpr int kRegCells = kRowsPerLane;
#ifndef MSW_LONG_STEP
#define MSW_LONG_STEP 8
#endif
constexpr int kLongStep = MSW_LONG_STEP;
#ifndef MSW_REVERSE_B
#define MSW_REVERSE_B true
#endif
#ifndef MSW_B_KEEPN
#define MSW_B_KEEPN MSW_REG_CELLS
#endif
#ifndef MSW_PASSA_BATCH
#define MSW_PASSA_BATCH 4
#endif
#ifdef MSW_NO_PRIME
constexpr bool kPrimeFirstSlice = false;
#else
constexpr bool kPrimeFirstSlice = true;
#endif
#ifndef MSW_PASSB_BATCH
#define MSW_PASSB_BATCH 4
#endif
#ifndef MSW_LONG_KEEP
#define MSW_LONG_KEEP 1
#endif
constexpr double kFxMagic = 6755399441055744.0;
constexpr unsigned long long kFxMagicBits = 0x4338000000000000ull;
__device__ __forceinline__ unsigned long long fx_bits(double scaled_r, double pk) {
  const double v = fma(scaled_r, pk, kFxMagic);
  const uint32_t hi = (uint32_t)__double2hiint(v) - (uint32_t)(kFxMagicBits >> 32);
  return ((unsigned long long)hi << 32) | (uint32_t)__double2loint(v);
}

#ifndef MSW_FAST_DIV
#define MSW_FAST_DIV 1
#endif
#ifndef MSW_DIV_CORRECT
#define MSW_DIV_CORRECT 0
#endif
__device__ __forceinline__ double ec_rcp(double z) {
#if MSW_FAST_DIV
  double r = __builtin_amdgcn_rcp(z);
  r = fma(fma(-z, r, 1.0), r, r);
  r = fma(fma(-z, r, 1.0), r, r);
  return r;
#else
  return 1.0 / z;
#endif
}
__device__ __forceinline__ double ec_div(double c, double z) {
#if MSW_FAST_DIV
  const double r = ec_rcp(z);
  const double q = c * r;
#if MSW_DIV_CORRECT
  return fma(fma(-z, q, c), r, q);
#else
  return q;
#endif
#else
  return c / z;
#endif
}

__device__ __forceinline__ uint32_t uniform(uint32_t v) { return __builtin_amdgcn_readfirstlane(v); }
__device__ __forceinline__ double uniform_d(double v) {
  const uint32_t lo = __builtin_amdgcn_readfirstlane(__double2loint(v));
  const uint32_t hi = __builtin_amdgcn_readfirstlane(__double2hiint(v));
  return __hiloint2double((int)hi, (int)lo);
}

template <int ENC, int RC = kRegCells>
struct SliceBuf {
  typename Rec<ENC>::T r[RC];
  typename Rec<ENC>::T rc[ENC == kEncIndex ? kColdRows : 1];
  uint32_t sl, o, len, nhot;
  uint32_t lgm, nec;
  uint32_t c8;
};

template <int ENC, int RC>
__device__ __forceinline__ void load_slice(const uint32_t *rec, size_t base, uint32_t len,
                                           typename Rec<ENC>::T (&r)[RC], typename Rec<ENC>::T nullr) {
#pragma unroll
  for (int k = 0; k < RC; k += 2) {
    if ((uint32_t)k < len) {
      r[k] = Rec<ENC>::load(rec, base + (size_t)k * 64);
      if constexpr (odd_slices(ENC)) {
        r[k + 1] = nullr;
        if ((uint32_t)k + 1 < len) r[k + 1] = Rec<ENC>::load(rec, base + (size_t)(k + 1) * 64);
      } else {
        r[k + 1] = Rec<ENC>::load(rec, base + (size_t)(k + 1) * 64);
      }
    }
  }
}
__device__ __forceinline__ void load_slice_split(const uint32_t *rec, size_t base, uint32_t len, uint32_t nhot,
                                                 uint32_t (&r)[kRegCells], uint32_t (&rc)[kColdRows], uint32_t nullr,
                                                 uint32_t nullr_hot) {
  const uint32_t ncold = len - nhot;
  if (ncold <= (uint32_t)kColdRows) {
    load_slice<kEncIndex>(rec, base, nhot, r, nullr_hot);
#pragma unroll
    for (int j = 0; j < kColdRows; ++j)
      if ((uint32_t)j < ncold) rc[j] = rec[base + (size_t)(nhot + j) * 64];
  } else {
    load_slice<kEncIndex>(rec, base, len, r, nullr);
  }
}

template <int ENC>
__device__ __forceinline__ typename Rec<ENC>::T null_record(uint32_t g, const RecDec &d, double tnull) {
  if constexpr (ENC == kEncValue) return ValRec{8u * g, tnull};
  else return Rec<ENC>::make(g, 0u, d);
}
#ifndef MSW_VAL_THREADS
#define MSW_VAL_THREADS 512
#endif
#ifndef MSW_HYB_THREADS_A
#define MSW_HYB_THREADS_A MSW_PASS_THREADS_A
#endif
template <int ENC>
constexpr int pass_threads_A() {
  return ENC == kEncValue ? MSW_VAL_THREADS : (ENC == kEncIndex ? MSW_HYB_THREADS_A : kPassThreads);
}
template <int ENC, int RC = kRegCells>
constexpr int pass_threads_B() { return ENC == kEncValue ? MSW_VAL_THREADS : (RC < kRegCells ? kPassThreadsB8 : kPassThreadsB); }

__device__ __forceinline__ void wait_vm0() { __builtin_amdgcn_s_waitcnt(0x0F70); }

#ifdef MSW_EXPERIMENT_NOSTREAM
#define MSW_REC_ROW(o) ((o) & 1023u)
#else
#define MSW_REC_ROW(o) (o)
#endif
template <int ENC, bool REVERSE, int RC = kRegCells>
struct SliceStream {
  const SellDev &S;
  uint32_t s_first, nw, n_mine, lane;
  uint32_t geo;
  typename Rec<ENC>::T nullr = {};
  typename Rec<ENC>::T nullr_hot = {};
  uint2 pend = make_uint2(0, 0);
  __device__ __forceinline__ SliceStream(const SellDev &S_, uint32_t first, uint32_t nw_, uint32_t lane_,
                                         uint32_t geo_)
      : S(S_), s_first(first), nw(nw_), lane(lane_), geo(geo_) {
    n_mine = first < S.nslices ? (S.nslices - first + nw_ - 1) / nw_ : 0;
    gather_offs(0);
  }
  __device__ __forceinline__ uint32_t slice_at(uint32_t i) const {
    return s_first + (REVERSE ? (i < n_mine ? n_mine - 1 - i : i) : i) * nw;
  }
  __device__ __forceinline__ void gather_offs(uint32_t chunk) {
    const uint32_t i = chunk * 64 + lane;
    pend = make_uint2(0, 0);
    if (i < n_mine) {
      const uint32_t sl = slice_at(i);
      const uint32_t o = S.slice_off[sl];
      const SliceGeo sg = slice_geo(S.cls, sl);
      pend = make_uint2(o, (S.slice_off[sl + 1] - o) | sg.lgm << kGeoLgmShift | sg.nec << kGeoNecShift);
      if constexpr (ENC == kEncIndex) pend.x |= (uint32_t)S.slice_hot[sl] << kGeoHotShift;
    }
  }
  __device__ __forceinline__ void commit_offs() {
    typedef uint32_t v2u_t __attribute__((ext_vector_type(2)));
    typedef __attribute__((address_space(3))) v2u_t lds_u2_t;
    v2u_t v = {pend.x, pend.y}, z = {0u, 0u};
    *(lds_u2_t *)(size_t)(geo + lane * 8) = v;
    if (lane < 2) *(lds_u2_t *)(size_t)(geo + (64 + lane) * 8) = z;
  }
  template <class Issue>
  __device__ __forceinline__ void fetch(uint32_t base, uint32_t j, SliceBuf<ENC, RC> &b, Issue &issue) {
    typedef uint32_t v2u_t __attribute__((ext_vector_type(2)));
    typedef __attribute__((address_space(3))) const v2u_t lds_cu2_t;
    const v2u_t oe = *(lds_cu2_t *)(size_t)(geo + j * 8);
    b.sl = slice_at(base + j);
    const uint32_t oy = uniform(oe.y);
    b.len = oy & ((1u << kGeoLgmShift) - 1u);
    b.lgm = (oy >> kGeoLgmShift) & 7u;
    b.nec = oy >> kGeoNecShift;
    if constexpr (ENC == kEncIndex) {
      const uint32_t ox = uniform(oe.x);
      b.o = ox & ((1u << kGeoHotShift) - 1u);
      b.nhot = ox >> kGeoHotShift;
      if (b.len <= (uint32_t)RC) load_slice_split(S.rec, (size_t)b.o * 64 + lane, b.len, b.nhot, b.r, b.rc, nullr, nullr_hot);
    } else {
      b.o = uniform(oe.x);
      if (b.len <= (uint32_t)RC) load_slice<ENC>(S.rec, (size_t)MSW_REC_ROW(b.o) * 64 + lane, b.len, b.r, nullr);
    }
    issue(b);
  }
  template <class Issue>
  __device__ __forceinline__ void prime(SliceBuf<ENC, RC> &first, Issue &issue) {
    commit_offs();
    fetch(0, 0, first, issue);
  }
  template <class Issue, class Process, class ChunkEnd>
  __device__ __forceinline__ void run(Issue issue, Process process, ChunkEnd chunk_end,
                                      const SliceBuf<ENC, RC> *primed = nullptr) {
    SliceBuf<ENC, RC> A = {}, B = {};
    if (primed) A = *primed;
    for (uint32_t base = 0; base == 0 || base < n_mine; base += 64) {
      if (base) gather_offs(base >> 6);
      if (base || !primed) commit_offs();
      const uint32_t n_chunk = n_mine > base ? (n_mine - base < 64u ? n_mine - base : 64u) : 0u;
      uint32_t j = 0;
      if (base || !primed) fetch(base, 0, A, issue);
      for (;;) {
        if (j >= n_chunk) break;
        wait_vm0();
        fetch(base, j + 1, B, issue);
        process(A);
        if (++j >= n_chunk) break;
        wait_vm0();
        fetch(base, j + 1, A, issue);
        process(B);
        ++j;
      }
      wait_vm0();
      chunk_end();
    }
  }
};

typedef double v2d_t __attribute__((ext_vector_type(2)));
typedef __attribute__((address_space(3))) const v2d_t lds_cd2_t;
typedef __attribute__((address_space(3))) const double lds_cd_t;
typedef __attribute__((address_space(3))) double lds_d_t;
template <bool INLDS>
__device__ __forceinline__ double2 tab16(const unsigned char *glob, uint32_t off) {
  if constexpr (INLDS) {
    const v2d_t v = *(lds_cd2_t *)(size_t)off;
    return make_double2(v.x, v.y);
  }
  else return *reinterpret_cast<const double2 *>(glob + off);
}
template <bool INLDS>
__device__ __forceinline__ double tab8(const unsigned char *glob, uint32_t off) {
  if constexpr (INLDS) return *(lds_cd_t *)(size_t)off;
  else return *reinterpret_cast<const double *>(glob + off);
}

struct AccA {
  double zs, t1, t2;
};
__device__ __forceinline__ void cellA(AccA &c, const double p0, const double e, const double w,
                                      const double x, const double D) {
  const double xm = x - p0;
  const double xD = x * D;
  const double wx = w * xm;
  c.zs = fma(e, xm, c.zs);
  c.t1 = fma(e, xD + wx, c.t1);
  c.t2 = fma(e, fma(xD, D, w * fma(2.0, xD, wx)), c.t2);
}

template <int ENC, bool GLDS, bool TLDS, bool ML>
__global__ __launch_bounds__(pass_threads_A<ENC>()) void k_passA(const Scalars *sc, SellDev S,
                                                       const double2 *ew_g, const double2 *tabA_g,
                                                       double *partA, const double *partR, int npartR, GuardDev GD) {
  extern __shared__ __align__(16) unsigned char smem[];
  using R = Rec<ENC>;
  using RT = typename R::T;
  constexpr bool HYB = ENC == kEncIndex;
  constexpr bool VAL = ENC == kEncValue;
  constexpr int NT = pass_threads_A<ENC>();
  static_assert(!((HYB || VAL) && TLDS), "index records go with the hybrid slot area, value records have no table");
  constexpr bool TL = TLDS || HYB;
  const RecDec D = rec_dec(S);
  const uint32_t n_tab = S.n_tab_lds;
  const int skip = sc->done;
  const int tid = threadIdx.x, lane = tid & 63;
  const uint32_t G = S.n_groups, Gp = G + kSentinels;
  const uint32_t bhiA = S.bhiA;
  const uint32_t scratch_off = (uint32_t)pass_scratch_off(GLDS ? 1 : 0, n_tab, G, true, HYB);
  double *sh = reinterpret_cast<double *>(smem + scratch_off);
  SliceStream<ENC, false> stream(S, uniform(blockIdx.x * (NT / 64) + (tid >> 6)),
                              gridDim.x * (NT / 64), (uint32_t)lane,
                              scratch_off + 256u + uniform(tid >> 6) * kGeoStride);
  [[maybe_unused]] const double vlogzi0 = uniform_d(sc->logzi);
  const RT null_rec = null_record<ENC>(S.n_groups + (uint32_t)lane, D, vlogzi0);
  stream.nullr = null_rec;
  if constexpr (HYB) stream.nullr_hot = R::make_h(S.n_groups + (uint32_t)lane, 0u, D);
  else stream.nullr_hot = null_rec;
  auto issue = [&](SliceBuf<ENC> &) {};
  constexpr bool PRIME = kPrimeFirstSlice && ENC == kEncNarrow;
  SliceBuf<ENC> first = {};
  if constexpr (PRIME) stream.prime(first, issue);
  double m1 = 0.0, m2 = 0.0;
  for (int b0 = 0; tid < 64 && b0 < npartR; b0 += 512) {
    double t1[8], t2[8];
#pragma unroll
    for (int k = 0; k < 8; ++k) {
      const int b = b0 + 64 * k + lane;
      t1[k] = b < npartR ? partR[kRedfinParts * b + 3] : 0.0;
      t2[k] = b < npartR ? partR[kRedfinParts * b + 4] : 0.0;
    }
#pragma unroll
    for (int k = 0; k < 8; ++k) m1 += t1[k], m2 += t2[k];
  }
  if (TL) {
    double2 *t = reinterpret_cast<double2 *>(smem);
    for (uint32_t i = tid; i < n_tab; i += NT) t[i] = tabA_g[i];
  }
  if (GLDS) {
    double2 *t = reinterpret_cast<double2 *>(smem + bhiA);
    for (uint32_t g = tid; g < Gp; g += NT) t[g] = ew_g[g];
  }
  const unsigned char *ew_b = reinterpret_cast<const unsigned char *>(ew_g) - bhiA;
  const unsigned char *xt_b = reinterpret_cast<const unsigned char *>(tabA_g);
  auto EW_ = [&](RT r) -> double2 { return tab16<GLDS>(ew_b, R::ew_off(r, D)); };
  auto EWh_ = [&](RT r) -> double2 { return tab16<GLDS>(ew_b, rec_ew_off<ENC, true>(r, D)); };
  [[maybe_unused]] const double va = uniform_d(sc->a), vtref = uniform_d(sc->tref), vlogzi = uniform_d(sc->logzi);
  [[maybe_unused]] const double voma = 1.0 - va;
  auto XTg_ = [&](RT r) -> double2 {
    if constexpr (VAL) return make_double2(exp_le0(va * (r.t - vtref)), voma * (r.t - vlogzi));
    else return tab16<TLDS>(xt_b, R::t_off(r, D));
  };
  auto XT_ = [&](RT r) -> double2 {
    if constexpr (VAL) return XTg_(r);
    else return tab16<TL>(xt_b, rec_t_off<ENC, true>(r, D));
  };
  const double p0 = uniform_d(sc->p0), U = uniform_d(sc->U);
  const double zbase = p0 * U;
  const double gthr = fmax(zbase * kGuardRatio, 2.2250738585072014e-308);
  const uint32_t gcnt_off = scratch_off + 128u;
  typedef __attribute__((address_space(3))) uint32_t lds_u32_t;
  auto defer = [&](uint32_t p) {
    const uint32_t i = __hip_atomic_fetch_add((lds_u32_t *)(size_t)gcnt_off, 1u, __ATOMIC_RELAXED, __HIP_MEMORY_SCOPE_WORKGROUP);
    if (i < GD.cap) GD.list[(size_t)blockIdx.x * GD.cap + i] = p;
    else *GD.err = 2;
  };
  double nn = 0.0;
  if (skip) return;
  if (tid == 0) *(lds_u32_t *)(size_t)gcnt_off = 0u;
  if (tid < 64) {
    m1 = wave_sum(m1);
    m2 = wave_sum(m2);
    if (tid == 0) sh[18] = m1, sh[19] = m2;
  }
  if (tid == 0 && blockIdx.x == 0) MSW_STAMP(sc->iter, 0, 0);
  __syncthreads();
  if (tid == 0 && blockIdx.x == 0) MSW_STAMP(sc->iter, 0, 1);
  const double b1 = p0 * uniform_d(sh[18]), b2 = p0 * uniform_d(sh[19]);

  auto process = [&](SliceBuf<ENC> &sb) {
    const uint32_t len = sb.len;
    AccA c = {0.0, 0.0, 0.0};
    auto fixed = [&](RT(&b)[kRegCells], auto LEN, auto ANY) {
      constexpr int L = decltype(LEN)::value;
      constexpr int B = MSW_PASSA_BATCH;
#pragma unroll
      for (int k0 = 0; k0 < L; k0 += B) {
        double2 ewv[B], xtv[B];
#pragma unroll
        for (int k = 0; k < B; ++k) {
          if (k0 + k < L) {
            if constexpr (decltype(ANY)::value) ewv[k] = EW_(b[k0 + k]), xtv[k] = XTg_(b[k0 + k]);
            else ewv[k] = EWh_(b[k0 + k]), xtv[k] = XT_(b[k0 + k]);
          }
        }
#pragma unroll
        for (int k = 0; k < B; ++k)
          if (k0 + k < L) cellA(c, p0, ewv[k].x, ewv[k].y, xtv[k].x, xtv[k].y);
      }
    };
    auto cells = [&](RT(&b)[kRegCells], uint32_t n) {
      n += n & 1;
      switch (n) {
        case 0: break;
        case 2: fixed(b, std::integral_constant<int, 2>{}, std::false_type{}); break;
        case 4: fixed(b, std::integral_constant<int, 4>{}, std::false_type{}); break;
        case 6: fixed(b, std::integral_constant<int, 6>{}, std::false_type{}); break;
#if MSW_REG_CELLS >= 12
        case 8: fixed(b, std::integral_constant<int, 8>{}, std::false_type{}); break;
        case 10: fixed(b, std::integral_constant<int, 10>{}, std::false_type{}); break;
#endif
#if MSW_REG_CELLS == 16
        case 12: fixed(b, std::integral_constant<int, 12>{}, std::false_type{}); break;
        case 14: fixed(b, std::integral_constant<int, 14>{}, std::false_type{}); break;
#endif
        default: fixed(b, std::integral_constant<int, kRegCells>{}, std::false_type{}); break;
      }
    };
    auto pairs_any = [&](RT(&b)[kRegCells], uint32_t n) {
#pragma unroll
      for (int k = 0; k < kRegCells; k += 2) {
        if ((uint32_t)k < n) {
          const double2 a0 = EW_(b[k]), a1 = EW_(b[k + 1]);
          const double2 x0 = XTg_(b[k]), x1 = XTg_(b[k + 1]);
          cellA(c, p0, a0.x, a0.y, x0.x, x0.y);
          cellA(c, p0, a1.x, a1.y, x1.x, x1.y);
        }
      }
    };
    if (len <= (uint32_t)kRegCells) {
      if constexpr (HYB) {
        const uint32_t nhot = sb.nhot, ncold = len - nhot;
        if (ncold <= (uint32_t)kColdRows) {
          double2 cew[kColdRows], cxt[kColdRows];
#pragma unroll
          for (int j = 0; j < kColdRows; ++j) {
            if ((uint32_t)j < ncold) {
              cxt[j] = XTg_(sb.rc[j]);
              cew[j] = EW_(sb.rc[j]);
            }
          }
          cells(sb.r, nhot);
#pragma unroll
          for (int j = 0; j < kColdRows; ++j)
            if ((uint32_t)j < ncold) cellA(c, p0, cew[j].x, cew[j].y, cxt[j].x, cxt[j].y);
        } else {
          pairs_any(sb.r, len);
        }
      } else {
        cells(sb.r, len);
      }
    } else {
      const size_t base = (size_t)sb.o * 64 + lane;
      RT t[kRegCells];
      uint32_t k0 = 0;
      for (; k0 + (uint32_t)kRegCells <= len; k0 += kRegCells) {
        load_slice<ENC>(S.rec, base + (size_t)k0 * 64, kRegCells, t, null_rec);
        fixed(t, std::integral_constant<int, kRegCells>{}, std::true_type{});
      }
      if (k0 < len) {
        const uint32_t n = len - k0;
        load_slice<ENC>(S.rec, base + (size_t)k0 * 64, n, t, null_rec);
        pairs_any(t, n);
      }
    }
    const uint32_t lgm = ML ? sb.lgm : 0u;
    bool mine = ((uint32_t)lane >> lgm) < sb.nec;
    if (ML && lgm != 0u) {
      c.zs = group_sum(c.zs, lgm);
      c.t1 = group_sum(c.t1, lgm);
      c.t2 = group_sum(c.t2, lgm);
      mine = mine && ((uint32_t)lane & ((1u << lgm) - 1u)) == 0u;
    }
    if (mine) {
      const double Zt = zbase + c.zs;
      if (Zt >= gthr) {
        const double iZ = ec_rcp(Zt);
        const double S1 = (b1 + c.t1) * iZ, S2 = (b2 + c.t2) * iZ;
        nn += S2 - S1 * S1;
      } else {
        defer(S.n_long + (ML ? slice_geo(S.cls, sb.sl).ec0 + ((uint32_t)lane >> lgm) : sb.sl * 64 + lane));
      }
    }
  };
  if constexpr (PRIME) stream.run(issue, process, [] {}, &first);
  else stream.run(issue, process, [] {});
  {
    constexpr int LS = ENC == kEncWide || VAL ? 4 : kLongStep;
    auto load_long = [&](uint32_t kb, uint32_t k1, RT(&dst)[LS]) {
#pragma unroll
      for (int u = 0; u < LS; ++u) {
        dst[u] = null_rec;
        if (kb + 64u * u < k1 && kb + 64u * u + lane < k1) dst[u] = R::load(S.rec_long, kb + 64u * u + lane);
      }
    };
    uint32_t r = stream.s_first, kb = 0, k1 = 0;
    bool have = r < S.n_long;
    if (have) kb = S.long_ptr[r], k1 = S.long_ptr[r + 1];
    RT cur[LS], nxt[LS];
    load_long(kb, k1, cur);
    AccA c = {0.0, 0.0, 0.0};
    while (have) {
      uint32_t nr = r, nkb = kb + LS * 64, nk1 = k1;
      bool nhave = true;
      if (nkb >= k1) {
        nr = r + stream.nw;
        nhave = nr < S.n_long;
        nkb = nk1 = 0;
        if (nhave) nkb = S.long_ptr[nr], nk1 = S.long_ptr[nr + 1];
      }
      load_long(nkb, nk1, nxt);
#pragma unroll
      for (int q = 0; q < LS; q += 4) {
        if (kb + 64u * q < k1) {
          double2 a0[4], x0[4];
#pragma unroll
          for (int u = 0; u < 4; ++u) a0[u] = EW_(cur[q + u]), x0[u] = XTg_(cur[q + u]);
#pragma unroll
          for (int u = 0; u < 4; ++u) cellA(c, p0, a0[u].x, a0[u].y, x0[u].x, x0[u].y);
        }
      }
      if (nr != r) {
        const double zs = wave_sum(c.zs), t1 = wave_sum(c.t1), t2 = wave_sum(c.t2);
        if (lane == 0) {
          const double Zt = zbase + zs;
          if (Zt >= gthr) {
            const double iZ = ec_rcp(Zt);
            const double S1 = (b1 + t1) * iZ, S2 = (b2 + t2) * iZ;
            nn += S2 - S1 * S1;
          } else {
            defer(r);
          }
        }
        c = {0.0, 0.0, 0.0};
      }
#pragma unroll
      for (int u = 0; u < LS; ++u) cur[u] = nxt[u];
      r = nr, kb = nkb, k1 = nk1, have = nhave;
    }
  }
  __syncthreads();
  const uint32_t n_guard = min(*(lds_u32_t *)(size_t)gcnt_off, GD.cap);
  if (n_guard) {
    const uint32_t wv = uniform(tid >> 6), nwv = NT / 64;
    uint32_t *bits = GD.bits + (size_t)(blockIdx.x * 16 + wv) * GD.words;
    const double a = uniform_d(sc->a), oma = 1.0 - a, logzi = uniform_d(sc->logzi), tref = uniform_d(sc->tref);
    for (uint32_t i = wv; i < n_guard; i += nwv) {
      const uint32_t p = GD.list[(size_t)blockIdx.x * GD.cap + i];
      double z = 0.0, t1 = 0.0, t2 = 0.0;
      wave_cells<ENC>(S, p, (uint32_t)lane, [&](uint32_t g, double T) {
        const double x = exp(a * (T - tref)), sv = oma * (T - logzi) + ew_g[g].y;
        const double q = ew_g[g].x * x;
        atomicOr(&bits[g >> 5], 1u << (g & 31));
        z += q;
        t1 = fma(q, sv, t1);
        t2 = fma(q * sv, sv, t2);
      });
      __builtin_amdgcn_s_waitcnt(0);
      for (uint32_t w0 = lane; w0 < GD.words; w0 += 64) {
        const uint32_t listed = atomicOr(&bits[w0], 0u);
        for (uint32_t b = 0; b < 32; ++b) {
          const uint32_t g = w0 * 32 + b;
          if (g < G && !((listed >> b) & 1u)) {
            const double2 ev = ew_g[g];
            const double q = ev.x * p0;
            z += q;
            t1 = fma(q, ev.y, t1);
            t2 = fma(q * ev.y, ev.y, t2);
          }
        }
        atomicAnd(&bits[w0], 0u);
      }
      z = wave_sum(z), t1 = wave_sum(t1), t2 = wave_sum(t2);
      if (lane == 0) {
        if (z > 0.0) {
          const double S1 = t1 / z, S2 = t2 / z;
          nn += S2 - S1 * S1;
        } else {
          *GD.err = 1;
        }
      }
      __builtin_amdgcn_s_waitcnt(0);
    }
  }
  nn = block_sum_fixed1<NT / 64>(nn, sh);
  if (tid == 0) MSW_STAMP_MAX(sc->iter, 0, 7);
  if (tid == 0) partA[blockIdx.x] = nn;
}

template <int ENC, int GMODE, bool TLDS, bool ML, int RC = kRegCells>
__global__ __launch_bounds__((pass_threads_B<ENC, RC>())) void k_passB(const Scalars *sc, SellDev S, const double *e_g,
                                                       const double2 *tabB_g, double *partAcc,
                                                       double *partS, double *accGlobal, RangeB rg, GuardDev GD) {
  extern __shared__ __align__(16) unsigned char smem[];
  using R = Rec<ENC>;
  using RT = typename R::T;
  constexpr bool HYB = ENC == kEncIndex;
  constexpr bool VAL = ENC == kEncValue;
  constexpr int NT = pass_threads_B<ENC, RC>();
  static_assert(!((HYB || VAL) && TLDS), "index records go with the hybrid slot area, value records have no table");
  constexpr bool TL = TLDS || HYB;
  const RecDec D = rec_dec(S);
  const uint32_t n_tab = S.n_tab_lds;
  const int skip = sc->done;
  const int tid = threadIdx.x, lane = tid & 63;
  const uint32_t G = S.n_groups, Gp = G + kSentinels;
  const uint32_t bhi = S.bhi;
  constexpr bool GLDS = GMODE == 1 || GMODE == 2;
  constexpr bool ALDS = GMODE > 0;
  const uint32_t acc_off = pass_acc_off(GMODE, G);
  const uint32_t scratch_off = (uint32_t)pass_scratch_off(GMODE, n_tab, G, false, HYB);
  double *sh = reinterpret_cast<double *>(smem + scratch_off);
  SliceStream<ENC, MSW_REVERSE_B, RC> stream(S, uniform(blockIdx.x * (NT / 64) + (tid >> 6)),
                              gridDim.x * (NT / 64), (uint32_t)lane,
                              scratch_off + 256u + uniform(tid >> 6) * kGeoStride);
  [[maybe_unused]] const double vlogzi0 = uniform_d(sc->logzi);
  const uint32_t n_lanes = S.nslices * 64u;
  const RT null_rec = null_record<ENC>(G + (uint32_t)lane, D, vlogzi0);
  stream.nullr = null_rec;
  if constexpr (HYB) stream.nullr_hot = R::make_h(G + (uint32_t)lane, 0u, D);
  else stream.nullr_hot = null_rec;
  auto issue = [&](SliceBuf<ENC, RC> &sb) {
    const uint32_t q = sb.sl * 64 + lane;
    const uint32_t cj = S.c8s[q < n_lanes ? q : 0u];
    sb.c8 = q < n_lanes ? cj : 0u;
  };
  constexpr bool PRIME = kPrimeFirstSlice && ENC == kEncNarrow && GMODE != 0 && GMODE != 3;
  SliceBuf<ENC, RC> first = {};
  if constexpr (PRIME) stream.prime(first, issue);
  if (TL) {
    double2 *t = reinterpret_cast<double2 *>(smem);
    for (uint32_t i = tid; i < n_tab; i += NT) t[i] = tabB_g[i];
  }
  if (ALDS) {
    double *el = reinterpret_cast<double *>(smem + bhi), *al = reinterpret_cast<double *>(smem + bhi + acc_off);
    const uint32_t n_acc = GMODE == 4 ? rg.n : Gp;
    for (uint32_t g = tid; g < n_acc; g += NT) {
      if (GLDS) el[g] = e_g[g];
      al[g] = 0.0;
    }
  }
  const unsigned char *e_b = reinterpret_cast<const unsigned char *>(e_g) - bhi;
  unsigned char *acc_b = reinterpret_cast<unsigned char *>(accGlobal) - bhi;
  const unsigned char *xt_b = reinterpret_cast<const unsigned char *>(tabB_g);
  auto E_ = [&](RT r) -> double { return tab8<GLDS>(e_b, R::e_off(r, D)); };
  auto Eh_ = [&](RT r) -> double { return tab8<GLDS>(e_b, rec_e_off<ENC, true>(r, D)); };
  [[maybe_unused]] const double va = uniform_d(sc->a), vtref = uniform_d(sc->tref), vlogzi = uniform_d(sc->logzi);
  [[maybe_unused]] const double vp0 = uniform_d(sc->p0), vp0l = vp0 * vlogzi;
  auto XTg_ = [&](RT r) -> double2 {
    if constexpr (VAL) {
      const double x = exp_le0(va * (r.t - vtref));
      return make_double2(x - vp0, fma(x, r.t, -vp0l));
    } else {
      return tab16<TLDS>(xt_b, R::t_off(r, D));
    }
  };
  auto XT_ = [&](RT r) -> double2 {
    if constexpr (VAL) return XTg_(r);
    else return tab16<TL>(xt_b, rec_t_off<ENC, true>(r, D));
  };
  auto XMg_ = [&](RT r) -> double {
    if constexpr (VAL) return exp_le0(va * (r.t - vtref)) - vp0;
    else return tab8<TLDS>(xt_b, R::t_off(r, D));
  };
  auto XMgh_ = [&](RT r) -> double {
    if constexpr (VAL) return exp_le0(va * (r.t - vtref)) - vp0;
    else return tab8<TLDS>(xt_b, rec_t_off<ENC, true>(r, D));
  };
  typedef __attribute__((address_space(3))) unsigned long long lds_u64_t;
  auto addACCx = [&](RT r, auto v, auto HOT) {
    using V = decltype(v);
    using LT = typename std::conditional<std::is_same<V, double>::value, lds_d_t, lds_u64_t>::type;
    const uint32_t off = rec_e_off<ENC, decltype(HOT)::value>(r, D);
    if constexpr (GMODE == 2)
      __hip_atomic_fetch_add((LT *)(size_t)(off + kAccFixed), v, __ATOMIC_RELAXED, __HIP_MEMORY_SCOPE_WORKGROUP);
    else if constexpr (GMODE == 1)
      __hip_atomic_fetch_add((LT *)(size_t)(off + acc_off), v, __ATOMIC_RELAXED, __HIP_MEMORY_SCOPE_WORKGROUP);
    else if constexpr (GMODE == 3)
      __hip_atomic_fetch_add((LT *)(size_t)off, v, __ATOMIC_RELAXED, __HIP_MEMORY_SCOPE_WORKGROUP);
    else if constexpr (GMODE == 4) {
      const uint32_t d = off - bhi - 8u * rg.g0;
      if (d < 8u * rg.n)
        __hip_atomic_fetch_add((LT *)(size_t)(bhi + d), v, __ATOMIC_RELAXED, __HIP_MEMORY_SCOPE_WORKGROUP);
    }
    else
      atomicAdd(reinterpret_cast<V *>(acc_b + off), v);
  };
  auto addACC = [&](RT r, auto v) { addACCx(r, v, std::false_type{}); };
  auto addFXx = [&](RT r, double rs, double pk, auto HOT) { addACCx(r, fx_bits(rs, pk), HOT); };
  auto addFXwidex = [&](RT r, double rs, double pk, auto HOT) {
    const double q = rs * pk;
    const double vh = fma(q, 0x1p-32, kFxMagic);
    const double qh = vh - kFxMagic;
    const double ql = fma(-qh, 0x1p32, q);
    addACCx(r, (unsigned long long)(uint32_t)__double2loint(vh) << 32, HOT);
    addACCx(r, fx_bits(1.0, ql), HOT);
  };
  auto addFX = [&](RT r, double rs, double pk) { addFXx(r, rs, pk, std::false_type{}); };
  auto addFXwide = [&](RT r, double rs, double pk) { addFXwidex(r, rs, pk, std::false_type{}); };
  const double p0 = uniform_d(sc->p0), U = uniform_d(sc->U);
  const double zbase = p0 * U, hbase = p0 * uniform_d(sc->logzi) * U;
  const int fxe = (int)uniform((uint32_t)fx_expbits(sc->fx_shift));
  const double fxs = uniform_d(sc->fx_scale), fxb = ldexp(uniform_d(sc->xb), 1 - (int)uniform((uint32_t)sc->fx_shift));
  const double fxt1 = 0x1p51 / fxs, fxt2 = 0x1p51 / (fxs * fxb);
  const double gthr = fmax(zbase * kGuardRatio, 2.2250738585072014e-308);
  const uint32_t gcnt_off = scratch_off + 128u;
  typedef __attribute__((address_space(3))) uint32_t lds_u32_t;
  auto defer = [&](uint32_t p) {
    const uint32_t i = __hip_atomic_fetch_add((lds_u32_t *)(size_t)gcnt_off, 1u, __ATOMIC_RELAXED, __HIP_MEMORY_SCOPE_WORKGROUP);
    if (i < GD.cap) GD.list[(size_t)blockIdx.x * GD.cap + i] = p;
    else *GD.err = 2;
  };
  double s_clogZ = 0.0, s_rH = 0.0, s_W = 0.0;
  double lp_mant = 1.0;
  int lp_exp = 0;
  auto flush_logs = [&] {
    s_clogZ += log(lp_mant) + (double)lp_exp * 0.693147180559945309417232121458;
    lp_mant = 1.0;
    lp_exp = 0;
  };
  if (skip) return;
  if (tid == 0) *(lds_u32_t *)(size_t)gcnt_off = 0u;
  if (tid == 0 && blockIdx.x == 0) MSW_STAMP(sc->iter, 2, 0);
  __syncthreads();
  if (tid == 0 && blockIdx.x == 0) MSW_STAMP(sc->iter, 2, 1);

  auto process = [&](SliceBuf<ENC, RC> &sb) {
    const uint32_t o = sb.o, len = sb.len;
    double c = (double)sb.c8;
    if (__builtin_amdgcn_ballot_w64(sb.c8 == kC8Escape)) {
      if (sb.c8 == kC8Escape)
        c = S.cvec[S.n_long + (ML ? slice_geo(S.cls, sb.sl).ec0 + ((uint32_t)lane >> sb.lgm) : sb.sl * 64 + lane)];
      __builtin_amdgcn_s_waitcnt(0x0F70);
    }
    double zs = 0.0, hs = 0.0;
    constexpr int KEEPN = ENC == kEncWide ? 4 : (MSW_B_KEEPN < RC ? MSW_B_KEEPN : RC);
    double xv[KEEPN > 0 ? KEEPN : 1];
    auto fixed = [&](RT(&b)[RC], auto LEN, auto KEEP, auto ANY) {
      constexpr int L = decltype(LEN)::value;
      constexpr bool KP = decltype(KEEP)::value;
      constexpr int B = MSW_PASSB_BATCH;
#pragma unroll
      for (int k0 = 0; k0 < L; k0 += B) {
        double ev[B];
        double2 xt[B];
#pragma unroll
        for (int k = 0; k < B; ++k) {
          if (k0 + k < L) {
            if constexpr (decltype(ANY)::value) ev[k] = E_(b[k0 + k]), xt[k] = XTg_(b[k0 + k]);
            else ev[k] = Eh_(b[k0 + k]), xt[k] = XT_(b[k0 + k]);
          }
        }
#pragma unroll
        for (int k = 0; k < B; ++k) {
          if (k0 + k < L) {
            zs = fma(ev[k], xt[k].x, zs);
            hs = fma(ev[k], xt[k].y, hs);
            if constexpr (KP && KEEPN > 0)
              if (k0 + k < KEEPN) xv[k0 + k] = kFx ? fx_factor(ev[k], fxe) * xt[k].x : xt[k].x;
          }
        }
      }
    };
    auto cells = [&](RT(&b)[RC], uint32_t n, auto KEEP) {
      n += n & 1;
      auto at_most = [&](auto N) {
        constexpr int L = decltype(N)::value < RC ? decltype(N)::value : RC;
        fixed(b, std::integral_constant<int, L>{}, KEEP, std::false_type{});
      };
      switch (n) {
        case 0: break;
        case 2: at_most(std::integral_constant<int, 2>{}); break;
        case 4: at_most(std::integral_constant<int, 4>{}); break;
        case 6: at_most(std::integral_constant<int, 6>{}); break;
        case 8: at_most(std::integral_constant<int, 8>{}); break;
        case 10: at_most(std::integral_constant<int, 10>{}); break;
        case 12: at_most(std::integral_constant<int, 12>{}); break;
        case 14: at_most(std::integral_constant<int, 14>{}); break;
        default: at_most(std::integral_constant<int, 16>{}); break;
      }
    };
    auto pairs_any = [&](RT(&b)[RC], uint32_t n) {
#pragma unroll
      for (int k = 0; k < RC; k += 2) {
        if ((uint32_t)k < n) {
          const double e0 = E_(b[k]), e1 = E_(b[k + 1]);
          const double2 t0 = XTg_(b[k]), t1 = XTg_(b[k + 1]);
          zs = fma(e0, t0.x, zs);
          hs = fma(e0, t0.y, hs);
          zs = fma(e1, t1.x, zs);
          hs = fma(e1, t1.y, hs);
        }
      }
    };
    auto scatter = [&](RT(&b)[RC], uint32_t n, double rj, auto KEPT, auto WIDE_ADD) {
      constexpr bool KP = decltype(KEPT)::value;
      constexpr bool WA = decltype(WIDE_ADD)::value;
#pragma unroll
      for (int k = 0; k < RC; k += 2) {
        if ((uint32_t)k < n) {
          double x0, x1;
          auto e_of = [&](RT r) { if constexpr (KP) return Eh_(r); else return E_(r); };
          auto xm_of = [&](RT r) { if constexpr (KP) return XMgh_(r); else return XMg_(r); };
          if constexpr (kFx) {
            x0 = KP && k < KEEPN ? xv[k < KEEPN ? k : 0] : fx_factor(e_of(b[k]), fxe) * xm_of(b[k]);
            x1 = KP && k + 1 < KEEPN ? xv[k + 1 < KEEPN ? k + 1 : 0] : fx_factor(e_of(b[k + 1]), fxe) * xm_of(b[k + 1]);
            if constexpr (WA) {
              addFXwidex(b[k], rj, x0, KEPT);
              addFXwidex(b[k + 1], rj, x1, KEPT);
            } else {
              addFXx(b[k], rj, x0, KEPT);
              addFXx(b[k + 1], rj, x1, KEPT);
            }
          } else {
            x0 = KP && k < KEEPN ? xv[k < KEEPN ? k : 0] : xm_of(b[k]);
            x1 = KP && k + 1 < KEEPN ? xv[k + 1 < KEEPN ? k + 1 : 0] : xm_of(b[k + 1]);
            addACCx(b[k], rj * x0, KEPT);
            addACCx(b[k + 1], rj * x1, KEPT);
          }
        }
      }
    };
    if (len <= (uint32_t)RC) {
      [[maybe_unused]] double xc[kColdRows];
      uint32_t nsc = len, ncold = 0;
      bool kept = true;
      if constexpr (HYB) {
        const uint32_t nhot = sb.nhot;
        if (len - nhot <= (uint32_t)kColdRows) {
          ncold = len - nhot;
          nsc = nhot;
          double ce[kColdRows];
          double2 cx[kColdRows];
#pragma unroll
          for (int j = 0; j < kColdRows; ++j) {
            if ((uint32_t)j < ncold) {
              cx[j] = XTg_(sb.rc[j]);
              ce[j] = E_(sb.rc[j]);
            }
          }
          cells(sb.r, nhot, std::true_type{});
#pragma unroll
          for (int j = 0; j < kColdRows; ++j) {
            if ((uint32_t)j < ncold) {
              zs = fma(ce[j], cx[j].x, zs);
              hs = fma(ce[j], cx[j].y, hs);
              xc[j] = kFx ? fx_factor(ce[j], fxe) * cx[j].x : cx[j].x;
            }
          }
        } else {
          pairs_any(sb.r, len);
          kept = false;
        }
      } else {
        cells(sb.r, len, std::true_type{});
      }
      auto scatter_all = [&](double rs, auto WIDE_ADD) {
        if (kept) scatter(sb.r, nsc, rs, std::true_type{}, WIDE_ADD);
        else scatter(sb.r, nsc, rs, std::false_type{}, WIDE_ADD);
        if constexpr (HYB) {
#pragma unroll
          for (int j = 0; j < kColdRows; ++j) {
            if ((uint32_t)j < ncold) {
              if constexpr (kFx) {
                if constexpr (decltype(WIDE_ADD)::value) addFXwide(sb.rc[j], rs, xc[j]);
                else addFX(sb.rc[j], rs, xc[j]);
              } else {
                addACC(sb.rc[j], rs * xc[j]);
              }
            }
          }
        }
      };
      const uint32_t lgm = ML ? sb.lgm : 0u;
      bool spoke = true;
      if (ML && lgm != 0u) {
        zs = group_sum(zs, lgm);
        hs = group_sum(hs, lgm);
        spoke = ((uint32_t)lane & ((1u << lgm) - 1u)) == 0u;
      }
      if (c != 0.0 && !(zbase + zs >= gthr)) {
        if (spoke) defer(S.n_long + (ML ? slice_geo(S.cls, sb.sl).ec0 + ((uint32_t)lane >> lgm) : sb.sl * 64 + lane));
      } else if (c != 0.0) {
        const double Z = zbase + zs;
        const double rj = ec_div(c, Z);
        double rja = rj;
        if (ML && lgm != 0u) rja = spoke ? rj : 0.0;
        s_rH = fma(rja, hs, s_rH);
        s_W += rja;
        if constexpr (kFx) {
          const double rs = rj * fxs;
          if (fma(rj, zbase, c) < fxt1 && rj < fxt2) scatter_all(rs, std::false_type{});
          else scatter_all(rs, std::true_type{});
        } else {
          scatter_all(rj, std::false_type{});
        }
        __builtin_amdgcn_sched_barrier(0);
        if (sb.c8 <= 15u) {
          const int ez = __builtin_amdgcn_frexp_exp(Z);
          const double m = __builtin_amdgcn_frexp_mant(Z);
          double r;
          if (__builtin_amdgcn_ballot_w64(sb.c8 > 3u) == 0) {
            r = m;
            r *= sb.c8 >= 2u ? m : 1.0;
            r *= sb.c8 >= 3u ? m : 1.0;
          } else {
            const double m2 = m * m, m4 = m2 * m2, m8 = m4 * m4;
            r = (sb.c8 & 1u) ? m : 1.0;
            r *= (sb.c8 & 2u) ? m2 : 1.0;
            r *= (sb.c8 & 4u) ? m4 : 1.0;
            r *= (sb.c8 & 8u) ? m8 : 1.0;
          }
          int ezc = __mul24(ez, (int)sb.c8);
          if (ML && lgm != 0u && !spoke) r = 1.0, ezc = 0;
          lp_mant *= r;
          lp_exp += ezc;
        } else if (spoke) {
          s_clogZ += c * log(Z);
        }
      }
    } else {
      const size_t base = (size_t)o * 64 + lane;
      RT t[RC];
      uint32_t k0 = 0;
      for (; k0 + (uint32_t)RC <= len; k0 += RC) {
        load_slice<ENC>(S.rec, base + (size_t)k0 * 64, RC, t, null_rec);
        fixed(t, std::integral_constant<int, RC>{}, std::false_type{}, std::true_type{});
      }
      if (k0 < len) {
        const uint32_t n = len - k0;
        load_slice<ENC>(S.rec, base + (size_t)k0 * 64, n, t, null_rec);
        pairs_any(t, n);
      }
      if (c != 0.0 && !(zbase + zs >= gthr)) {
        defer(S.n_long + (ML ? slice_geo(S.cls, sb.sl).ec0 : sb.sl * 64) + lane);
      } else if (c != 0.0) {
        const double Z = zbase + zs;
        const double rj = ec_div(c, Z);
        s_clogZ += c * log(Z);
        s_rH = fma(rj, hs, s_rH);
        s_W += rj;
        const double rs = kFx ? rj * fxs : rj;
        const bool narrow = !kFx || (fma(rj, zbase, c) < fxt1 && rj < fxt2);
        for (k0 = 0; k0 < len; k0 += RC) {
          const uint32_t n = len - k0 < (uint32_t)RC ? len - k0 : (uint32_t)RC;
          load_slice<ENC>(S.rec, base + (size_t)k0 * 64, n, t, null_rec);
          if (narrow) scatter(t, n, rs, std::false_type{}, std::false_type{});
          else scatter(t, n, rs, std::false_type{}, std::true_type{});
        }
      }
    }
  };
  if constexpr (PRIME) stream.run(issue, process, flush_logs, &first);
  else stream.run(issue, process, flush_logs);
  {
    uint32_t r = stream.s_first, c0 = 0, c1 = 0;
    if (r < S.n_long) c0 = S.long_ptr[r], c1 = S.long_ptr[r + 1];
    auto load_long = [&](uint32_t kb, uint32_t k1, RT(&dst)[kLongStep]) {
#pragma unroll
      for (int u = 0; u < kLongStep; ++u) {
        dst[u] = null_rec;
        if (kb + 64u * u < k1 && kb + 64u * u + lane < k1) dst[u] = R::load(S.rec_long, kb + 64u * u + lane);
      }
    };
    RT pre[kLongStep];
    load_long(c0, c1, pre);
    uint32_t n_deferred = 0;
    while (r < S.n_long) {
      const uint32_t rn = r + stream.nw;
      uint32_t n0 = 0, n1 = 0;
      if (rn < S.n_long) n0 = S.long_ptr[rn], n1 = S.long_ptr[rn + 1];
      const double c = S.cvec[r];
      RT first[kLongStep], rc[kLongStep];
#pragma unroll
      for (int u = 0; u < kLongStep; ++u) first[u] = rc[u] = pre[u];
      load_long(n0, n1, pre);
      double zs = 0.0, hs = 0.0;
      double pkf[kLongStep];
      for (uint32_t kb = c0;;) {
#pragma unroll
        for (int q = 0; q < kLongStep; q += 4) {
          if (kb + 64u * q < c1) {
            double eg[4];
            double2 t[4];
#pragma unroll
            for (int u = 0; u < 4; ++u) eg[u] = E_(rc[q + u]), t[u] = XTg_(rc[q + u]);
#pragma unroll
            for (int u = 0; u < 4; ++u) {
              zs = fma(eg[u], t[u].x, zs);
              hs = fma(eg[u], t[u].y, hs);
            }
#if MSW_LONG_KEEP
            if (kb == c0) {
#pragma unroll
              for (int u = 0; u < 4; ++u) pkf[q + u] = kFx ? fx_factor(eg[u], fxe) * t[u].x : t[u].x;
            }
#endif
          }
        }
        kb += kLongStep * 64;
        if (kb >= c1) break;
        load_long(kb, c1, rc);
      }
      zs = wave_sum(zs);
      hs = wave_sum(hs);
      if (c != 0.0 && !(zbase + zs >= gthr)) {
        if (lane == 0) defer(r);
      } else if (c != 0.0) {
        const double Z = zbase + zs;
        const double rj = ec_div(c, Z);
        const uint32_t c8l = uniform((uint32_t)S.c8[r]);
        if (c8l <= 15u) {
          if (lane == 0) {
            int ez;
            const double m = frexp(Z, &ez);
            const double m2 = m * m, m4 = m2 * m2, m8 = m4 * m4;
            double pw = (c8l & 1u) ? m : 1.0;
            pw *= (c8l & 2u) ? m2 : 1.0;
            pw *= (c8l & 4u) ? m4 : 1.0;
            pw *= (c8l & 8u) ? m8 : 1.0;
            lp_mant *= pw;
            lp_exp += ez * (int)c8l;
          }
          if (++n_deferred == 32u) {
            flush_logs();
            n_deferred = 0;
          }
        } else if (lane == 0) {
          s_clogZ += c * log(Z);
        }
        if (lane == 0) {
          s_rH = fma(rj, hs, s_rH);
          s_W += rj;
        }
#pragma unroll
        for (int u = 0; u < kLongStep; ++u) rc[u] = first[u];
        const double rs = kFx ? rj * fxs : rj;
        const bool narrow = !kFx || (fma(rj, zbase, c) < fxt1 && rj < fxt2);
        for (uint32_t kb = c0;;) {
#pragma unroll
          for (int q = 0; q < kLongStep; q += 4) {
            if (kb + 64u * q < c1) {
              double xm[4];
              if (MSW_LONG_KEEP && kb == c0) {
#pragma unroll
                for (int u = 0; u < 4; ++u) xm[u] = pkf[q + u];
              } else {
#pragma unroll
                for (int u = 0; u < 4; ++u) xm[u] = kFx ? fx_factor(E_(rc[q + u]), fxe) * XMg_(rc[q + u]) : XMg_(rc[q + u]);
              }
#pragma unroll
              for (int u = 0; u < 4; ++u) {
                if constexpr (kFx) {
                  if (narrow) addFX(rc[q + u], rs, xm[u]);
                  else addFXwide(rc[q + u], rs, xm[u]);
                } else {
                  addACC(rc[q + u], rj * xm[u]);
                }
              }
            }
          }
          kb += kLongStep * 64;
          if (kb >= c1) break;
          load_long(kb, c1, rc);
        }
      }
      r = rn, c0 = n0, c1 = n1;
    }
    flush_logs();
  }
  __syncthreads();
  const uint32_t n_guard = (GMODE != 4 || rg.first) ? min(*(lds_u32_t *)(size_t)gcnt_off, GD.cap) : 0u;
  if (n_guard) {
    if (tid == 0) atomicAdd(GD.visits, (unsigned long long)n_guard);
    const uint32_t wv = uniform(tid >> 6), nwv = NT / 64;
    uint32_t *bits = GD.bits + (size_t)(blockIdx.x * 16 + wv) * GD.words;
    const double a = uniform_d(sc->a), logzi = uniform_d(sc->logzi), tref = uniform_d(sc->tref);
    const double tls = uniform_d(sc->fx_tscale);
    auto add_share = [&](uint32_t g, double share) {
      const double vh = fma(share, tls, kFxMagic);
      const double qh = vh - kFxMagic;
      const double ql = fma(share, tls, -qh) * 0x1p36;
      atomicAdd(&GD.tail[2 * (size_t)g], fx_bits(1.0, qh));
      atomicAdd(&GD.tail[2 * (size_t)g + 1], fx_bits(1.0, ql));
    };
    for (uint32_t i = wv; i < n_guard; i += nwv) {
      const uint32_t p = GD.list[(size_t)blockIdx.x * GD.cap + i];
      const double c = S.cvec[p];
      double z = 0.0, h = 0.0;
      wave_cells<ENC>(S, p, (uint32_t)lane, [&](uint32_t g, double T) {
        const double q = e_g[g] * exp(a * (T - tref));
        atomicOr(&bits[g >> 5], 1u << (g & 31));
        z += q;
        h = fma(q, T, h);
      });
      __builtin_amdgcn_s_waitcnt(0);
      double r0 = 0.0;
      for (uint32_t w0 = lane; w0 < GD.words; w0 += 64) {
        const uint32_t listed = atomicOr(&bits[w0], 0u);
        for (uint32_t b = 0; b < 32; ++b) {
          const uint32_t g = w0 * 32 + b;
          if (g < G && !((listed >> b) & 1u)) r0 += e_g[g];
        }
      }
      z = wave_sum(z), h = wave_sum(h), r0 = wave_sum(r0);
      const double Z = fma(p0, r0, z), H = fma(p0 * logzi, r0, h);
      if (Z > 0.0) {
        const double rj = c / Z;
        if (lane == 0) {
          s_clogZ += c * log(Z);
          s_rH += rj * H;
        }
        wave_cells<ENC>(S, p, (uint32_t)lane, [&](uint32_t g, double T) {
          add_share(g, e_g[g] * rj * exp(a * (T - tref)));
        });
        for (uint32_t w0 = lane; w0 < GD.words; w0 += 64) {
          const uint32_t listed = atomicAnd(&bits[w0], 0u);
          for (uint32_t b = 0; b < 32; ++b) {
            const uint32_t g = w0 * 32 + b;
            if (g < G && !((listed >> b) & 1u)) add_share(g, e_g[g] * (rj * p0));
          }
        }
      } else {
        if (lane == 0) *GD.err = 1;
        for (uint32_t w0 = lane; w0 < GD.words; w0 += 64) atomicAnd(&bits[w0], 0u);
      }
      __builtin_amdgcn_s_waitcnt(0);
    }
  }
  s_rH = fma(hbase, s_W, s_rH);
  {
    double t3[3] = {s_clogZ, s_rH, s_W};
    block_sum_n<3>(t3, sh + 32);
    if (tid == 0 && (GMODE != 4 || rg.first)) {
      partS[4 * blockIdx.x + 0] = t3[0];
      partS[4 * blockIdx.x + 1] = t3[1];
      partS[4 * blockIdx.x + 2] = t3[2];
      partS[4 * blockIdx.x + 3] = 0.0;
    }
  }
  if (tid == 0) MSW_STAMP_MAX(sc->iter, 2, 6);
  if (ALDS) {
    __syncthreads();
    const double *al = reinterpret_cast<const double *>(smem + bhi + acc_off);
    double *dst = partAcc + (size_t)blockIdx.x * G;
    if (GMODE == 4) {
      for (uint32_t g = tid; g < rg.n; g += NT) dst[rg.g0 + g] = al[g];
    } else {
      for (uint32_t g = tid; g < G; g += NT) dst[g] = al[g];
    }
  }
  if (tid == 0) MSW_STAMP_MAX(sc->iter, 2, 7);
}

}
```

Baseline: 225200 billion.

## Move bound's entropy term from pass B into pass A and shrink B table to 8 bytes

The H (entropy) accumulation used for the bound is computed in pass A, which already has the per-read normaliser, instead of in pass B. Pass B then drops the hs accumulation and reads an 8-byte table entry rather than a 16-byte double2, which cuts memory traffic and FMAs in the hot loop. finstep gains a split variant that combines the pass A partial sum with an analytic logzi term. Thread counts and batch sizes for the wide and narrow encodings are retuned, and the final pass A before an eval is reused to skip one pass A on resume. The cost is extra work in pass A (one more accumulator plus a per-slice multiplicity load) and a reformulation of the bound that may differ numerically.

```diff
diff --git a/msweep_amd/csrc/common.hpp b/msweep_amd/csrc/common.hpp
--- a/msweep_amd/csrc/common.hpp
+++ b/msweep_amd/csrc/common.hpp
@@ -22,6 +22,10 @@
 constexpr int kPassThreads = MSW_PASS_THREADS_A;
 constexpr int kPassThreadsB = MSW_PASS_THREADS_B;
 constexpr int kPassThreadsB8 = MSW_PASS_THREADS_B8;
+#ifndef MSW_B_TAB8
+#define MSW_B_TAB8 1
+#endif
+constexpr bool kTab8 = MSW_B_TAB8 != 0;
 constexpr int kMaxTrace = 4096;
 constexpr int kRedfinParts = 5;
 constexpr int kRedfinGroups = 16;
@@ -97,6 +101,10 @@
 
 struct TabDev {
   double2 *A, *B;
+  __device__ __forceinline__ void storeB(int i, double xm) const {
+    if constexpr (kTab8) reinterpret_cast<double *>(B)[i] = xm;
+    else B[i] = make_double2(xm, 0.0);
+  }
 };
 
 struct Scalars {
diff --git a/msweep_amd/csrc/msweep_core.hip b/msweep_amd/csrc/msweep_core.hip
--- a/msweep_amd/csrc/msweep_core.hip
+++ b/msweep_amd/csrc/msweep_core.hip
@@ -111,6 +111,7 @@
   DevBuf<int32_t> tr_reset;
   bool have_solution = false;
   bool prepared = false;
+  bool passA_current = false;
   int last_algo = MSW_ALGO_RCG;
   DevBuf<double> logth;
   DevBuf<float> e32, tab32;
@@ -381,11 +382,12 @@
   s.tabB.alloc((size_t)std::max<uint32_t>(L.n_area, 1));
   s.tab_built.alloc(2);
   const int nb = std::max(L.nblk, std::max(L.nblk_dense, L.npart_rows()));
-  s.partA.alloc(std::max(nb, 1024));
+  s.partA.alloc(2 * (size_t)std::max(nb, 1024));
+  s.passA_current = false;
   s.partS.alloc(4 * (size_t)std::max(nb, 1024));
   s.partR.alloc(kRedfinParts * ((size_t)G / kRedfinGroups + 2));
   s.totS.alloc(4);
-  s.commA.alloc(1);
+  s.commA.alloc(2);
   s.commB.alloc(3 * (size_t)G + 4);
   s.partAcc.alloc((size_t)std::max(nb, 1) * G);
   s.partC.alloc(1024);
@@ -647,6 +649,24 @@
                      s.tab_built.p);
 }
 
+bool bound_split(const Resident &L) { return L.flavor == 0 && L.enc != kEncValue; }
+
+void launch_passA_reduced(const Resident &L, Solver &s) {
+  launch_passA(L, s);
+  if (s.comm()) {
+    std::pair<hipEvent_t, hipEvent_t> *evc = nullptr;
+    if (s.profiling) {
+      evc = &next_pair(s.evC, s.evC_used);
+      MSW_HIP(hipEventRecord(evc->first, s.stream));
+    }
+    const int nbA = L.flavor == 0 ? L.nblk : L.nblk_dense;
+    const int nsums = bound_split(L) ? 2 : 1;
+    hipLaunchKernelGGL(k_sum_scalar, dim3(1), dim3(1024), 0, s.stream, s.sc.p, 1, nbA, nsums, s.partA.p, s.commA.p);
+    s.comm()->allreduce(s.commA.p, (size_t)nsums, s.stream);
+    if (evc) MSW_HIP(hipEventRecord(evc->second, s.stream));
+  }
+}
+
 void launch_finstep(const Resident &L, Solver &s, int mode) {
   TraceDev tr{s.tr_bound.p, s.tr_newnorm.p, s.tr_beta.p, s.tr_theta.p, s.tr_reset.p};
   const double *pA = s.partA.p;
@@ -655,7 +675,8 @@
     pA = s.commA.p;
     npA = 1;
   }
-  hipLaunchKernelGGL(k_finstep, dim3(1), dim3(1024), 0, s.stream, s.sc.p, mode, (int)L.G, L.n_tab_inline(), npA, pA,
+  hipLaunchKernelGGL(bound_split(L) ? k_finstep<true> : k_finstep<false>, dim3(1), dim3(1024), 0, s.stream, s.sc.p, mode,
+                     (int)L.G, L.n_tab_inline(), npA, pA,
                      (int)((L.G + kRedfinGroups - 1) / kRedfinGroups), s.totS.p, s.partR.p, s.Nc.p, s.w.p, s.u.p,
                      s.os_u.p, s.step_u.p, L.lut_area.p, s.e.p, s.tabs(), tr);
   launch_tables(L, s);
@@ -693,6 +714,7 @@
   MSW_HIP(hipGetLastError());
   MSW_HIP(hipStreamSynchronize(s.stream));
   s.prepared = true;
+  s.passA_current = false;
 }
 
 void validate_solve(size_t max_iters, int algo, int prec) {
@@ -704,12 +726,13 @@
 
 void begin_solve(const Resident &L, Solver &s, double tol, size_t max_iters) {
   const uint32_t G = L.G;
+  s.passA_current = false;
   if (s.trace_theta) s.tr_theta.alloc(s.trace_theta * G);
   const double *cpart = s.partC.p;
   int ncpart = kCvecBlocks;
   if (s.comm()) {
     s.comm()->rendezvous();
-    hipLaunchKernelGGL(k_sum_scalar, dim3(1), dim3(1024), 0, s.stream, s.sc.p, 0, kCvecBlocks, s.partC.p,
+    hipLaunchKernelGGL(k_sum_scalar, dim3(1), dim3(1024), 0, s.stream, s.sc.p, 0, kCvecBlocks, 1, s.partC.p,
                        s.commA.p);
     s.comm()->allreduce(s.commA.p, 1, s.stream);
     cpart = s.commA.p;
@@ -733,24 +756,15 @@
     s.timing.passB_launches--;
     if (s.profiling && s.evB_used) s.evB_used--;
   }
-  const int nbA = L.flavor == 0 ? L.nblk : L.nblk_dense;
+  bool skip_passA = iters_start > 0 && s.passA_current;
+  s.passA_current = false;
   size_t iters_done = iters_start;
   for (;;) {
     const size_t missing = std::max<size_t>(1, max_iters - std::min(max_iters, iters_done));
     const size_t batch = s.fixed_iters ? std::min<size_t>(256, missing) : std::min<size_t>(kIterBatch, missing);
     for (size_t b = 0; b < batch; ++b) {
-      launch_passA(L, s);
-      if (s.comm()) {
-        std::pair<hipEvent_t, hipEvent_t> *evc = nullptr;
-        if (s.profiling) {
-          evc = &next_pair(s.evC, s.evC_used);
-          MSW_HIP(hipEventRecord(evc->first, s.stream));
-        }
-        hipLaunchKernelGGL(k_sum_scalar, dim3(1), dim3(1024), 0, s.stream, s.sc.p, 1, nbA, s.partA.p,
-                           s.commA.p);
-        s.comm()->allreduce(s.commA.p, 1, s.stream);
-        if (evc) MSW_HIP(hipEventRecord(evc->second, s.stream));
-      }
+      if (!skip_passA) launch_passA_reduced(L, s);
+      skip_passA = false;
       launch_finstep(L, s, 0);
       launch_passB(L, s);
     }
@@ -758,9 +772,11 @@
     poll(s);
     if (s.sc_host->done) break;
     if (s.sc_host->have_eval && (size_t)s.sc_host->iter + 1 >= max_iters) {
+      if (bound_split(L)) launch_passA_reduced(L, s);
       launch_finstep(L, s, 1);
       MSW_HIP(hipGetLastError());
       poll(s);
+      s.passA_current = bound_split(L) && !s.sc_host->reset_pending;
       if (s.sc_host->done) break;
     }
     iters_done = (size_t)s.sc_host->iter;
diff --git a/msweep_amd/csrc/state_kernels.hpp b/msweep_amd/csrc/state_kernels.hpp
--- a/msweep_amd/csrc/state_kernels.hpp
+++ b/msweep_amd/csrc/state_kernels.hpp
@@ -28,7 +28,7 @@
   for (int i = tid; i < n_lut; i += nt) {
     const double T = lut[i], x = exp(a * (T - tref));
     X.A[i] = make_double2(x, oma * (T - logzi));
-    X.B[i] = make_double2(x - p0, x * T - p0 * logzi);
+    X.storeB(i, x - p0);
   }
   if (tid == 0) {
     sc->M = M;
@@ -52,7 +52,7 @@
     for (int i = blockIdx.x * blockDim.x + threadIdx.x; i < n_tab; i += gridDim.x * blockDim.x) {
       const double T = lut[i], x = exp(a * (T - tref));
       X.A[i] = make_double2(x, oma * (T - logzi));
-      X.B[i] = make_double2(x - p0, x * T - p0 * logzi);
+      X.storeB(i, x - p0);
     }
   }
   __syncthreads();
@@ -96,6 +96,7 @@
 }
 
 constexpr int kStepRegs = 6;
+template <bool SPLIT>
 __global__ __launch_bounds__(1024) void k_finstep(Scalars *sc, int mode, int G, int n_lut, int n_partA,
                                                  const double *partA, int npartR, const double *totS,
                                                  const double *partR, const double *Nc, const double *w, double *u,
@@ -104,10 +105,14 @@
   __shared__ double sh[16 * (kRedfinParts + 1)];
   const int tid = threadIdx.x, nt = blockDim.x;
   const bool inreg = G <= kStepRegs * nt;
+  constexpr int kQH = 4;
   double q[kRedfinParts + 1] = {0.0, 0.0, 0.0, 0.0, 0.0, 0.0};
   for (int b = tid; b < npartR; b += nt)
-    for (int i = 0; i < kRedfinParts; ++i) q[i] += partR[kRedfinParts * b + i];
+    for (int i = 0; i < kRedfinParts; ++i)
+      if (!(SPLIT && i == kQH)) q[i] += partR[kRedfinParts * b + i];
   for (int i = tid; i < n_partA; i += nt) q[kRedfinParts] += partA[i];
+  if constexpr (SPLIT)
+    for (int i = tid; i < n_partA; i += nt) q[kQH] += partA[n_partA + i];
   const double s_clogZ = totS[0], s_rH = totS[1];
   double wv[kStepRegs], sv[kStepRegs], uv[kStepRegs];
   if (inreg) {
@@ -139,7 +144,12 @@
   } else if (s0.have_eval == 1) {
     const int reeval = s0.reset_pending;
     const double coef = (flavor == 0) ? (1.0 - a) : 1.0;
-    const double nb = s0.bound_const + s_clogZ + coef * s_rH + mu + lg + (flavor == 0 ? a * s0.tref * s0.csum : 0.0);
+    double nb;
+    if constexpr (SPLIT)
+      nb = s0.bound_const + s_clogZ + (coef * s_rH + q[kQH] + (1.0 - a) * logzi * s0.csum) + mu + lg +
+           a * s0.tref * s0.csum;
+    else
+      nb = s0.bound_const + s_clogZ + coef * s_rH + mu + lg + (flavor == 0 ? a * s0.tref * s0.csum : 0.0);
     if (!reeval && nb < s0.oldbound) {
       double a2 = a;
       if (s0.beta > 0) {
@@ -277,7 +287,7 @@
     for (int i = tid; i < n_lut; i += nt) {
       const double T = i == tid ? lt : lut[i], x = exp(a_new * (T - tref));
       X.A[i] = make_double2(x, oma * (T - logzi));
-      X.B[i] = make_double2(x - p0, x * T - p0 * logzi);
+      X.storeB(i, x - p0);
     }
   }
   double M = 0.0, U = 0.0;
@@ -457,14 +467,16 @@
   }
 }
 
-__global__ __launch_bounds__(1024) void k_sum_scalar(const Scalars *sc, int gate, int n, const double *part,
+__global__ __launch_bounds__(1024) void k_sum_scalar(const Scalars *sc, int gate, int n, int nsums, const double *part,
                                                     double *out) {
   __shared__ double sh[32];
   if (gate && sc->done) return;
-  double p = 0.0;
-  for (int i = threadIdx.x; i < n; i += blockDim.x) p += part[i];
-  p = block_sum(p, sh);
-  if (threadIdx.x == 0) out[0] = p;
+  for (int k = 0; k < nsums; ++k) {
+    double p = 0.0;
+    for (int i = threadIdx.x; i < n; i += blockDim.x) p += part[(size_t)k * n + i];
+    p = block_sum(p, sh);
+    if (threadIdx.x == 0) out[k] = p;
+  }
 }
 
 __global__ __launch_bounds__(1024) void k_colsum(const Scalars *sc, int G, int nrows, int fxrows, int npartS,
diff --git a/msweep_amd/csrc/sweep_kernels.hpp b/msweep_amd/csrc/sweep_kernels.hpp
--- a/msweep_amd/csrc/sweep_kernels.hpp
+++ b/msweep_amd/csrc/sweep_kernels.hpp
@@ -27,6 +27,9 @@
 #endif
 #ifndef MSW_PASSB_BATCH
 #define MSW_PASSB_BATCH 4
+#endif
+#ifndef MSW_PASSB_BATCH_T
+#define MSW_PASSB_BATCH_T 2
 #endif
 #ifndef MSW_LONG_KEEP
 #define MSW_LONG_KEEP 1
@@ -126,12 +129,33 @@
 #ifndef MSW_HYB_THREADS_A
 #define MSW_HYB_THREADS_A MSW_PASS_THREADS_A
 #endif
+#ifndef MSW_WIDE_THREADS_A
+#define MSW_WIDE_THREADS_A 512
+#endif
+#ifndef MSW_WIDE_THREADS_B
+#define MSW_WIDE_THREADS_B 512
+#endif
+#ifndef MSW_WIDE_KEEPN
+#define MSW_WIDE_KEEPN 4
+#endif
 template <int ENC>
 constexpr int pass_threads_A() {
-  return ENC == kEncValue ? MSW_VAL_THREADS : (ENC == kEncIndex ? MSW_HYB_THREADS_A : kPassThreads);
-}
+  return ENC == kEncValue ? MSW_VAL_THREADS
+                          : (ENC == kEncIndex ? MSW_HYB_THREADS_A : (ENC == kEncWide ? MSW_WIDE_THREADS_A : kPassThreads));
+}
+#ifndef MSW_PASS_THREADS_BN
+#define MSW_PASS_THREADS_BN MSW_PASS_THREADS_B
+#endif
+#ifndef MSW_B_KEEPN_N
+#define MSW_B_KEEPN_N MSW_B_KEEPN
+#endif
 template <int ENC, int RC = kRegCells>
-constexpr int pass_threads_B() { return ENC == kEncValue ? MSW_VAL_THREADS : (RC < kRegCells ? kPassThreadsB8 : kPassThreadsB); }
+constexpr int pass_threads_B() {
+  return ENC == kEncValue ? MSW_VAL_THREADS
+                          : (RC < kRegCells ? kPassThreadsB8
+                                            : (ENC == kEncNarrow ? MSW_PASS_THREADS_BN
+                                                                 : (ENC == kEncWide ? MSW_WIDE_THREADS_B : kPassThreadsB)));
+}
 
 __device__ __forceinline__ void wait_vm0() { __builtin_amdgcn_s_waitcnt(0x0F70); }
 
@@ -249,6 +273,7 @@
 
 struct AccA {
   double zs, t1, t2;
+  double h;
 };
 __device__ __forceinline__ void cellA(AccA &c, const double p0, const double e, const double w,
                                       const double x, const double D) {
@@ -258,6 +283,7 @@
   c.zs = fma(e, xm, c.zs);
   c.t1 = fma(e, xD + wx, c.t1);
   c.t2 = fma(e, fma(xD, D, w * fma(2.0, xD, wx)), c.t2);
+  c.h = fma(e, xD, c.h);
 }
 
 template <int ENC, bool GLDS, bool TLDS, bool ML>
@@ -269,6 +295,7 @@
   using RT = typename R::T;
   constexpr bool HYB = ENC == kEncIndex;
   constexpr bool VAL = ENC == kEncValue;
+  constexpr bool SPLIT = !VAL;
   constexpr int NT = pass_threads_A<ENC>();
   static_assert(!((HYB || VAL) && TLDS), "index records go with the hybrid slot area, value records have no table");
   constexpr bool TL = TLDS || HYB;
@@ -288,7 +315,14 @@
   stream.nullr = null_rec;
   if constexpr (HYB) stream.nullr_hot = R::make_h(S.n_groups + (uint32_t)lane, 0u, D);
   else stream.nullr_hot = null_rec;
-  auto issue = [&](SliceBuf<ENC> &) {};
+  const uint32_t n_lanes = S.nslices * 64u;
+  auto issue = [&](SliceBuf<ENC> &sb) {
+    if constexpr (SPLIT) {
+      const uint32_t q = sb.sl * 64 + lane;
+      const uint32_t cj = S.c8s[q < n_lanes ? q : 0u];
+      sb.c8 = q < n_lanes ? cj : 0u;
+    }
+  };
   constexpr bool PRIME = kPrimeFirstSlice && ENC == kEncNarrow;
   SliceBuf<ENC> first = {};
   if constexpr (PRIME) stream.prime(first, issue);
@@ -336,7 +370,7 @@
     if (i < GD.cap) GD.list[(size_t)blockIdx.x * GD.cap + i] = p;
     else *GD.err = 2;
   };
-  double nn = 0.0;
+  double nn = 0.0, sH = 0.0;
   if (skip) return;
   if (tid == 0) *(lds_u32_t *)(size_t)gcnt_off = 0u;
   if (tid < 64) {
@@ -351,7 +385,7 @@
 
   auto process = [&](SliceBuf<ENC> &sb) {
     const uint32_t len = sb.len;
-    AccA c = {0.0, 0.0, 0.0};
+    AccA c = {0.0, 0.0, 0.0, 0.0};
     auto fixed = [&](RT(&b)[kRegCells], auto LEN, auto ANY) {
       constexpr int L = decltype(LEN)::value;
       constexpr int B = MSW_PASSA_BATCH;
@@ -441,7 +475,17 @@
       c.zs = group_sum(c.zs, lgm);
       c.t1 = group_sum(c.t1, lgm);
       c.t2 = group_sum(c.t2, lgm);
+      if constexpr (SPLIT) c.h = group_sum(c.h, lgm);
       mine = mine && ((uint32_t)lane & ((1u << lgm) - 1u)) == 0u;
+    }
+    [[maybe_unused]] double cm = 0.0;
+    if constexpr (SPLIT) {
+      cm = (double)sb.c8;
+      if (__builtin_amdgcn_ballot_w64(sb.c8 == kC8Escape)) {
+        if (sb.c8 == kC8Escape)
+          cm = S.cvec[S.n_long + (ML ? slice_geo(S.cls, sb.sl).ec0 + ((uint32_t)lane >> lgm) : sb.sl * 64 + lane)];
+        __builtin_amdgcn_s_waitcnt(0x0F70);
+      }
     }
     if (mine) {
       const double Zt = zbase + c.zs;
@@ -449,6 +493,7 @@
         const double iZ = ec_rcp(Zt);
         const double S1 = (b1 + c.t1) * iZ, S2 = (b2 + c.t2) * iZ;
         nn += S2 - S1 * S1;
+        if constexpr (SPLIT) sH = fma(cm * iZ, c.h, sH);
       } else {
         defer(S.n_long + (ML ? slice_geo(S.cls, sb.sl).ec0 + ((uint32_t)lane >> lgm) : sb.sl * 64 + lane));
       }
@@ -469,8 +514,12 @@
     bool have = r < S.n_long;
     if (have) kb = S.long_ptr[r], k1 = S.long_ptr[r + 1];
     RT cur[LS], nxt[LS];
+    [[maybe_unused]] double cl = 0.0, cln = 0.0;
+    if constexpr (SPLIT) {
+      if (have) cl = S.cvec[r];
+    }
     load_long(kb, k1, cur);
-    AccA c = {0.0, 0.0, 0.0};
+    AccA c = {0.0, 0.0, 0.0, 0.0};
     while (have) {
       uint32_t nr = r, nkb = kb + LS * 64, nk1 = k1;
       bool nhave = true;
@@ -479,6 +528,9 @@
         nhave = nr < S.n_long;
         nkb = nk1 = 0;
         if (nhave) nkb = S.long_ptr[nr], nk1 = S.long_ptr[nr + 1];
+        if constexpr (SPLIT) {
+          if (nhave) cln = S.cvec[nr];
+        }
       }
       load_long(nkb, nk1, nxt);
 #pragma unroll
@@ -493,17 +545,21 @@
       }
       if (nr != r) {
         const double zs = wave_sum(c.zs), t1 = wave_sum(c.t1), t2 = wave_sum(c.t2);
+        [[maybe_unused]] double hw = 0.0;
+        if constexpr (SPLIT) hw = wave_sum(c.h);
         if (lane == 0) {
           const double Zt = zbase + zs;
           if (Zt >= gthr) {
             const double iZ = ec_rcp(Zt);
             const double S1 = (b1 + t1) * iZ, S2 = (b2 + t2) * iZ;
             nn += S2 - S1 * S1;
+            if constexpr (SPLIT) sH = fma(cl * iZ, hw, sH);
           } else {
             defer(r);
           }
         }
-        c = {0.0, 0.0, 0.0};
+        c = {0.0, 0.0, 0.0, 0.0};
+        cl = cln;
       }
 #pragma unroll
       for (int u = 0; u < LS; ++u) cur[u] = nxt[u];
@@ -519,10 +575,12 @@
     for (uint32_t i = wv; i < n_guard; i += nwv) {
       const uint32_t p = GD.list[(size_t)blockIdx.x * GD.cap + i];
       double z = 0.0, t1 = 0.0, t2 = 0.0;
+      [[maybe_unused]] double hg = 0.0;
       wave_cells<ENC>(S, p, (uint32_t)lane, [&](uint32_t g, double T) {
         const double x = exp(a * (T - tref)), sv = oma * (T - logzi) + ew_g[g].y;
         const double q = ew_g[g].x * x;
         atomicOr(&bits[g >> 5], 1u << (g & 31));
+        if constexpr (SPLIT) hg = fma(q, oma * (T - logzi), hg);
         z += q;
         t1 = fma(q, sv, t1);
         t2 = fma(q * sv, sv, t2);
@@ -543,10 +601,15 @@
         atomicAnd(&bits[w0], 0u);
       }
       z = wave_sum(z), t1 = wave_sum(t1), t2 = wave_sum(t2);
+      if constexpr (SPLIT) hg = wave_sum(hg);
       if (lane == 0) {
         if (z > 0.0) {
           const double S1 = t1 / z, S2 = t2 / z;
           nn += S2 - S1 * S1;
+          if constexpr (SPLIT) {
+            const double cg = S.cvec[p];
+            if (cg != 0.0) sH = fma(cg, hg / z, sH);
+          }
         } else {
           *GD.err = 1;
         }
@@ -554,9 +617,13 @@
       __builtin_amdgcn_s_waitcnt(0);
     }
   }
-  nn = block_sum_fixed1<NT / 64>(nn, sh);
+  double t2[2] = {nn, sH};
+  block_sum_fixed<2, NT / 64>(t2, sh + 32);
   if (tid == 0) MSW_STAMP_MAX(sc->iter, 0, 7);
-  if (tid == 0) partA[blockIdx.x] = nn;
+  if (tid == 0) {
+    partA[blockIdx.x] = t2[0];
+    partA[gridDim.x + blockIdx.x] = SPLIT ? t2[1] : 0.0;
+  }
 }
 
 template <int ENC, int GMODE, bool TLDS, bool ML, int RC = kRegCells>
@@ -568,6 +635,7 @@
   using RT = typename R::T;
   constexpr bool HYB = ENC == kEncIndex;
   constexpr bool VAL = ENC == kEncValue;
+  constexpr bool SPLIT = !VAL;
   constexpr int NT = pass_threads_B<ENC, RC>();
   static_assert(!((HYB || VAL) && TLDS), "index records go with the hybrid slot area, value records have no table");
   constexpr bool TL = TLDS || HYB;
@@ -600,8 +668,14 @@
   SliceBuf<ENC, RC> first = {};
   if constexpr (PRIME) stream.prime(first, issue);
   if (TL) {
-    double2 *t = reinterpret_cast<double2 *>(smem);
-    for (uint32_t i = tid; i < n_tab; i += NT) t[i] = tabB_g[i];
+    if constexpr (kTab8 && SPLIT) {
+      double *t = reinterpret_cast<double *>(smem);
+      const double *src = reinterpret_cast<const double *>(tabB_g);
+      for (uint32_t i = tid; i < n_tab; i += NT) t[i] = src[i];
+    } else {
+      double2 *t = reinterpret_cast<double2 *>(smem);
+      for (uint32_t i = tid; i < n_tab; i += NT) t[i] = tabB_g[i];
+    }
   }
   if (ALDS) {
     double *el = reinterpret_cast<double *>(smem + bhi), *al = reinterpret_cast<double *>(smem + bhi + acc_off);
@@ -618,25 +692,40 @@
   auto Eh_ = [&](RT r) -> double { return tab8<GLDS>(e_b, rec_e_off<ENC, true>(r, D)); };
   [[maybe_unused]] const double va = uniform_d(sc->a), vtref = uniform_d(sc->tref), vlogzi = uniform_d(sc->logzi);
   [[maybe_unused]] const double vp0 = uniform_d(sc->p0), vp0l = vp0 * vlogzi;
+  [[maybe_unused]] const uint32_t tw = D.mask ? (uint32_t)__builtin_popcount(D.mask) - 1u : 0u;
+  [[maybe_unused]] const uint32_t twH = D.maskH ? (uint32_t)__builtin_popcount(D.maskH) - 1u : 0u;
+  auto xoff = [&](RT r) -> uint32_t {
+    if constexpr (VAL) return 0u;
+    else if constexpr (!kTab8) return R::t_off(r, D);
+    else if constexpr (HYB) return (r & D.mask) << 3;
+    else if constexpr (ENC == kEncNarrow) return __builtin_amdgcn_ubfe(r, 1u, tw);
+    else return R::t_off(r, D) >> 1;
+  };
+  auto xoff_h = [&](RT r) -> uint32_t {
+    if constexpr (VAL) return 0u;
+    else if constexpr (!kTab8) return rec_t_off<ENC, true>(r, D);
+    else if constexpr (HYB) return __builtin_amdgcn_ubfe(r, 1u, twH);
+    else return xoff(r);
+  };
   auto XTg_ = [&](RT r) -> double2 {
     if constexpr (VAL) {
       const double x = exp_le0(va * (r.t - vtref));
       return make_double2(x - vp0, fma(x, r.t, -vp0l));
     } else {
-      return tab16<TLDS>(xt_b, R::t_off(r, D));
+      return make_double2(tab8<TLDS>(xt_b, xoff(r)), 0.0);
     }
   };
   auto XT_ = [&](RT r) -> double2 {
     if constexpr (VAL) return XTg_(r);
-    else return tab16<TL>(xt_b, rec_t_off<ENC, true>(r, D));
+    else return make_double2(tab8<TL>(xt_b, xoff_h(r)), 0.0);
   };
   auto XMg_ = [&](RT r) -> double {
     if constexpr (VAL) return exp_le0(va * (r.t - vtref)) - vp0;
-    else return tab8<TLDS>(xt_b, R::t_off(r, D));
+    else return tab8<TLDS>(xt_b, xoff(r));
   };
   auto XMgh_ = [&](RT r) -> double {
     if constexpr (VAL) return exp_le0(va * (r.t - vtref)) - vp0;
-    else return tab8<TLDS>(xt_b, rec_t_off<ENC, true>(r, D));
+    else return tab8<TLDS>(xt_b, xoff_h(r));
   };
   typedef __attribute__((address_space(3))) unsigned long long lds_u64_t;
   auto addACCx = [&](RT r, auto v, auto HOT) {
@@ -670,7 +759,8 @@
   auto addFX = [&](RT r, double rs, double pk) { addFXx(r, rs, pk, std::false_type{}); };
   auto addFXwide = [&](RT r, double rs, double pk) { addFXwidex(r, rs, pk, std::false_type{}); };
   const double p0 = uniform_d(sc->p0), U = uniform_d(sc->U);
-  const double zbase = p0 * U, hbase = p0 * uniform_d(sc->logzi) * U;
+  const double zbase = p0 * U;
+  [[maybe_unused]] const double hbase = SPLIT ? 0.0 : p0 * uniform_d(sc->logzi) * U;
   const int fxe = (int)uniform((uint32_t)fx_expbits(sc->fx_shift));
   const double fxs = uniform_d(sc->fx_scale), fxb = ldexp(uniform_d(sc->xb), 1 - (int)uniform((uint32_t)sc->fx_shift));
   const double fxt1 = 0x1p51 / fxs, fxt2 = 0x1p51 / (fxs * fxb);
@@ -698,19 +788,24 @@
 
   auto process = [&](SliceBuf<ENC, RC> &sb) {
     const uint32_t o = sb.o, len = sb.len;
-    double c = (double)sb.c8;
-    if (__builtin_amdgcn_ballot_w64(sb.c8 == kC8Escape)) {
-      if (sb.c8 == kC8Escape)
-        c = S.cvec[S.n_long + (ML ? slice_geo(S.cls, sb.sl).ec0 + ((uint32_t)lane >> sb.lgm) : sb.sl * 64 + lane)];
-      __builtin_amdgcn_s_waitcnt(0x0F70);
-    }
-    double zs = 0.0, hs = 0.0;
-    constexpr int KEEPN = ENC == kEncWide ? 4 : (MSW_B_KEEPN < RC ? MSW_B_KEEPN : RC);
+    auto mult = [&]() -> double {
+      double cj = (double)sb.c8;
+      if (__builtin_amdgcn_ballot_w64(sb.c8 == kC8Escape)) {
+        if (sb.c8 == kC8Escape)
+          cj = S.cvec[S.n_long + (ML ? slice_geo(S.cls, sb.sl).ec0 + ((uint32_t)lane >> sb.lgm) : sb.sl * 64 + lane)];
+        __builtin_amdgcn_s_waitcnt(0x0F70);
+      }
+      return cj;
+    };
+    double zs = 0.0;
+    [[maybe_unused]] double hs = 0.0;
+    constexpr int KEEPN0 = ENC == kEncNarrow ? MSW_B_KEEPN_N : MSW_B_KEEPN;
+    constexpr int KEEPN = ENC == kEncWide ? MSW_WIDE_KEEPN : (KEEPN0 < RC ? KEEPN0 : RC);
     double xv[KEEPN > 0 ? KEEPN : 1];
     auto fixed = [&](RT(&b)[RC], auto LEN, auto KEEP, auto ANY) {
       constexpr int L = decltype(LEN)::value;
       constexpr bool KP = decltype(KEEP)::value;
-      constexpr int B = MSW_PASSB_BATCH;
+      constexpr int B = VAL ? MSW_PASSB_BATCH : MSW_PASSB_BATCH_T;
 #pragma unroll
       for (int k0 = 0; k0 < L; k0 += B) {
         double ev[B];
@@ -726,7 +821,7 @@
         for (int k = 0; k < B; ++k) {
           if (k0 + k < L) {
             zs = fma(ev[k], xt[k].x, zs);
-            hs = fma(ev[k], xt[k].y, hs);
+            if constexpr (!SPLIT) hs = fma(ev[k], xt[k].y, hs);
             if constexpr (KP && KEEPN > 0)
               if (k0 + k < KEEPN) xv[k0 + k] = kFx ? fx_factor(ev[k], fxe) * xt[k].x : xt[k].x;
           }
@@ -758,9 +853,9 @@
           const double e0 = E_(b[k]), e1 = E_(b[k + 1]);
           const double2 t0 = XTg_(b[k]), t1 = XTg_(b[k + 1]);
           zs = fma(e0, t0.x, zs);
-          hs = fma(e0, t0.y, hs);
+          if constexpr (!SPLIT) hs = fma(e0, t0.y, hs);
           zs = fma(e1, t1.x, zs);
-          hs = fma(e1, t1.y, hs);
+          if constexpr (!SPLIT) hs = fma(e1, t1.y, hs);
         }
       }
     };
@@ -815,7 +910,7 @@
           for (int j = 0; j < kColdRows; ++j) {
             if ((uint32_t)j < ncold) {
               zs = fma(ce[j], cx[j].x, zs);
-              hs = fma(ce[j], cx[j].y, hs);
+              if constexpr (!SPLIT) hs = fma(ce[j], cx[j].y, hs);
               xc[j] = kFx ? fx_factor(ce[j], fxe) * cx[j].x : cx[j].x;
             }
           }
@@ -847,9 +942,10 @@
       bool spoke = true;
       if (ML && lgm != 0u) {
         zs = group_sum(zs, lgm);
-        hs = group_sum(hs, lgm);
+        if constexpr (!SPLIT) hs = group_sum(hs, lgm);
         spoke = ((uint32_t)lane & ((1u << lgm) - 1u)) == 0u;
       }
+      const double c = mult();
       if (c != 0.0 && !(zbase + zs >= gthr)) {
         if (spoke) defer(S.n_long + (ML ? slice_geo(S.cls, sb.sl).ec0 + ((uint32_t)lane >> lgm) : sb.sl * 64 + lane));
       } else if (c != 0.0) {
@@ -857,7 +953,7 @@
         const double rj = ec_div(c, Z);
         double rja = rj;
         if (ML && lgm != 0u) rja = spoke ? rj : 0.0;
-        s_rH = fma(rja, hs, s_rH);
+        if constexpr (!SPLIT) s_rH = fma(rja, hs, s_rH);
         s_W += rja;
         if constexpr (kFx) {
           const double rs = rj * fxs;
@@ -903,13 +999,14 @@
         load_slice<ENC>(S.rec, base + (size_t)k0 * 64, n, t, null_rec);
         pairs_any(t, n);
       }
+      const double c = mult();
       if (c != 0.0 && !(zbase + zs >= gthr)) {
         defer(S.n_long + (ML ? slice_geo(S.cls, sb.sl).ec0 : sb.sl * 64) + lane);
       } else if (c != 0.0) {
         const double Z = zbase + zs;
         const double rj = ec_div(c, Z);
         s_clogZ += c * log(Z);
-        s_rH = fma(rj, hs, s_rH);
+        if constexpr (!SPLIT) s_rH = fma(rj, hs, s_rH);
         s_W += rj;
         const double rs = kFx ? rj * fxs : rj;
         const bool narrow = !kFx || (fma(rj, zbase, c) < fxt1 && rj < fxt2);
@@ -946,7 +1043,8 @@
 #pragma unroll
       for (int u = 0; u < kLongStep; ++u) first[u] = rc[u] = pre[u];
       load_long(n0, n1, pre);
-      double zs = 0.0, hs = 0.0;
+      double zs = 0.0;
+      [[maybe_unused]] double hs = 0.0;
       double pkf[kLongStep];
       for (uint32_t kb = c0;;) {
 #pragma unroll
@@ -959,7 +1057,7 @@
 #pragma unroll
             for (int u = 0; u < 4; ++u) {
               zs = fma(eg[u], t[u].x, zs);
-              hs = fma(eg[u], t[u].y, hs);
+              if constexpr (!SPLIT) hs = fma(eg[u], t[u].y, hs);
             }
 #if MSW_LONG_KEEP
             if (kb == c0) {
@@ -974,7 +1072,7 @@
         load_long(kb, c1, rc);
       }
       zs = wave_sum(zs);
-      hs = wave_sum(hs);
+      if constexpr (!SPLIT) hs = wave_sum(hs);
       if (c != 0.0 && !(zbase + zs >= gthr)) {
         if (lane == 0) defer(r);
       } else if (c != 0.0) {
@@ -1001,7 +1099,7 @@
           s_clogZ += c * log(Z);
         }
         if (lane == 0) {
-          s_rH = fma(rj, hs, s_rH);
+          if constexpr (!SPLIT) s_rH = fma(rj, hs, s_rH);
           s_W += rj;
         }
 #pragma unroll
@@ -1058,12 +1156,13 @@
     for (uint32_t i = wv; i < n_guard; i += nwv) {
       const uint32_t p = GD.list[(size_t)blockIdx.x * GD.cap + i];
       const double c = S.cvec[p];
-      double z = 0.0, h = 0.0;
+      double z = 0.0;
+      [[maybe_unused]] double h = 0.0;
       wave_cells<ENC>(S, p, (uint32_t)lane, [&](uint32_t g, double T) {
         const double q = e_g[g] * exp(a * (T - tref));
         atomicOr(&bits[g >> 5], 1u << (g & 31));
         z += q;
-        h = fma(q, T, h);
+        if constexpr (!SPLIT) h = fma(q, T, h);
       });
       __builtin_amdgcn_s_waitcnt(0);
       double r0 = 0.0;
@@ -1074,13 +1173,15 @@
           if (g < G && !((listed >> b) & 1u)) r0 += e_g[g];
         }
       }
-      z = wave_sum(z), h = wave_sum(h), r0 = wave_sum(r0);
-      const double Z = fma(p0, r0, z), H = fma(p0 * logzi, r0, h);
+      z = wave_sum(z), r0 = wave_sum(r0);
+      if constexpr (!SPLIT) h = wave_sum(h);
+      const double Z = fma(p0, r0, z);
+      [[maybe_unused]] const double H = SPLIT ? 0.0 : fma(p0 * logzi, r0, h);
       if (Z > 0.0) {
         const double rj = c / Z;
         if (lane == 0) {
           s_clogZ += c * log(Z);
-          s_rH += rj * H;
+          if constexpr (!SPLIT) s_rH += rj * H;
         }
         wave_cells<ENC>(S, p, (uint32_t)lane, [&](uint32_t g, double T) {
           add_share(g, e_g[g] * rj * exp(a * (T - tref)));
@@ -1099,7 +1200,7 @@
       __builtin_amdgcn_s_waitcnt(0);
     }
   }
-  s_rH = fma(hbase, s_W, s_rH);
+  if constexpr (!SPLIT) s_rH = fma(hbase, s_W, s_rH);
   {
     double t3[3] = {s_clogZ, s_rH, s_W};
     block_sum_n<3>(t3, sh + 32);
```

Result: slower. 222900 billion (-1.0%).
